# xXCoffeeColaXc/WeatherConverter

Hardware: NVIDIA B200
Metric: guided translation images/sec (256x512, T steps) at 1/2/4/8 B200 vs host CPU (higher is better)
Workload: dtype bf16

## Files before the change

### include/wc_b200.h

```cpp
#ifndef WC_B200_H_
#define WC_B200_H_

#include <stddef.h>
#include <stdint.h>

#ifdef __cplusplus
extern "C" {
#endif

typedef uint16_t wc_bf16;

const char* wc_last_error(void);
int wc_abi_version(void);
long long wc_launch_count(void);

void wc_profile_begin(void);
int wc_profile_end(double* ms_by_class, long long* count_by_class, double* work_by_class);
int wc_profile_detail(int cap, int* cls, double* ms, double* work, int* info);

int wc_ddpm_step(const float* xt, const float* eps, const float* z, float* out, float* mean_out, float* sigz_out,
                 size_t n_per_sample, int batch, float beta, float sqrt_one_minus_acp, float sqrt_alpha, float sigma,
                 void* stream);
int wc_ddpm_step_batched(const float* xt, const float* eps, const float* z, float* out, float* mean_out,
                         float* sigz_out, size_t n_per_sample, int batch, const float* betas, const float* alphas,
                         const float* sqrt_one_minus_acp, const int64_t* t, int num_timesteps, void* stream);
int wc_ddpm_step_indexed(const float* xt, const float* eps, const float* z, float* out, float* mean_out, float* sigz_out,
                         size_t n_per_sample, int batch, const float* coef_tables, const int64_t* t_dev, int num_timesteps,
                         void* stream);
int wc_ddim_step(const float* xt, const float* eps, const float* z, float* out, float* mean_out, float* sigz_out,
                 size_t n_per_sample, int batch, float a_t, float s_t, float a_prev, float d, float sigma, void* stream);
int wc_ddim_step_indexed(const float* xt, const float* eps, const float* z, float* out, float* mean_out, float* sigz_out,
                         size_t n_per_sample, int batch, const float* coef_tables, const int64_t* t_dev, int num_timesteps,
                         void* stream);
int wc_add_noise(const float* x0, const float* noise, float* out, size_t n_per_sample, int batch,
                 const float* sqrt_acp, const float* sqrt_one_minus_acp, const int64_t* t, int num_timesteps, void* stream);

int wc_set_time_factor_table(const float* factor_host, int half);
int wc_time_embedding(const int64_t* t, int n, int dim, float* out, void* stream);

int wc_sgg_update(const float* grad, const float* mu, const float* sigz, float* out, float* mag_out, int batch, int h,
                  int w, int pool, float lambda, void* stream);

int wc_lcg_prepare(const float* sr_xt, const int64_t* gt, float* x_masked, int64_t* gt_masked, int batch, int num_classes,
                   int H, int W, void* stream);
int wc_lcg_combine(const float* pooled_grads, const int64_t* gt, const float* mu, const float* sigz, float* out, int batch,
                   int num_classes, int h, int w, int pool, float lambda, void* stream);

size_t wc_groupnorm_workspace_bytes(int batch);
int wc_groupnorm_silu(const wc_bf16* x, wc_bf16* y, int batch, int hw, int channels, int ldx, int ldy,
                      const float* gamma, const float* beta, float eps, int silu, void* workspace, void* stream);
int wc_conv2d(const wc_bf16* x, int batch, int H, int W, int Cin, int ldx, const float* weight, const float* bias,
              int Cout, int K, int stride, int pad, int dil, int transposed, const float* rowbias,
              const wc_bf16* residual, int ldr, const wc_bf16* x2, int Cin2, int ldx2, const float* weight2, int relu,
              wc_bf16* y, int ldy, void* stream);
int wc_conv_in(const float* x, const float* weight, const float* bias, const float* scale, const float* shift,
               wc_bf16* y, int batch, int H, int W, int Cout, int K, int stride, int pad, int ldy, int relu,
               void* stream);
int wc_conv_out(const wc_bf16* x, const float* weight, const float* bias, float* y, int batch, int H, int W, int Cin,
                int K, int ldx, int tanh_out, void* stream);
int wc_conv2d_dgrad(const wc_bf16* dz, int batch, int Ho, int Wo, int Cout, const float* weight, int Cin, int K, int stride,
                    int dil, const wc_bf16* residual, const wc_bf16* mask, wc_bf16* dx, void* stream);
int wc_maxpool3x3s2(const wc_bf16* x, wc_bf16* y, uint8_t* idx, int batch, int H, int W, int C, void* stream);
int wc_maxpool3x3s2_bwd(const wc_bf16* dy, const uint8_t* idx, const wc_bf16* x, wc_bf16* dx, int batch, int H, int W, int C,
                        void* stream);
int wc_bilinear(const wc_bf16* x, wc_bf16* y, int batch, int Hi, int Wi, int Ho, int Wo, int C, void* stream);
int wc_bilinear_bwd(const wc_bf16* dy, const wc_bf16* mask, wc_bf16* dx, int batch, int Hi, int Wi, int Ho, int Wo, int C,
                    void* stream);
int wc_seg_loss_head(const float* logits_lo, const int64_t* labels, int* n_valid_ws, int64_t* pred, float* dlogit_hi,
                     float* loss, float* logits_hi, wc_bf16* dlogit_lo, int batch, int h, int w, int H, int W, void* stream);
int wc_conv1_dgrad(const wc_bf16* dz, const float* weight, const float* scale, float* dx, int batch, int H, int W, void* stream);
int wc_nchw_f32_to_nhwc_bf16(const float* x, wc_bf16* y, int batch, int C, int hw, int ldy, void* stream);
int wc_nhwc_bf16_to_nchw_f32(const wc_bf16* x, float* y, int batch, int C, int hw, int ldx, void* stream);
int wc_attention(const wc_bf16* q, const wc_bf16* k, const wc_bf16* vt, wc_bf16* out, int batch, int heads, int ntok,
                 int hd, int ldo, void* stream);
int wc_attention_scaled(const wc_bf16* q, const wc_bf16* k, const wc_bf16* vt, wc_bf16* out, int batch, int heads, int ntok,
                        int hd, int ldo, float scale, void* stream);

int wc_ddpm_grid_u8(const float* x, uint8_t* out, int batch, int H, int W, int nrow, int padding, void* stream);
int wc_postprocess_u8(const float* x, uint8_t* out, int batch, int H, int W, const float* mean3_host, const float* std3_host, void* stream);
int wc_label_encode(const uint8_t* label_ids, int Ws, const int* ytab, const int* xtab, int top, int left, int Hc, int Wc,
                    const int64_t* lut, int nlut, int64_t* out, void* stream);
int wc_resample_u8(const uint8_t* in, uint8_t* tmp, uint8_t* out, int Hin, int Win, int Hout, int Wout, int channels, const int* bounds_h,
                   const int* kk_h, int ksize_h, const int* bounds_v, const int* kk_v, int ksize_v, void* stream);
int wc_u8_to_tensor(const uint8_t* in, int Win, int top, int left, int Hc, int Wc, int mode, const float* mean3_host, const float* std3_host,
                    float* out, void* stream);

int wc_attention_lse(const wc_bf16* q, const wc_bf16* k, const wc_bf16* vt, wc_bf16* out, float* lse, int batch, int heads,
                     int ntok, int hd, int ldo, void* stream);
int wc_attention_bwd(const wc_bf16* q, const wc_bf16* k, const wc_bf16* v, const wc_bf16* o, const wc_bf16* d_o, const float* lse,
                     float* d_scratch, wc_bf16* dqkv, int batch, int heads, int ntok, int hd, void* stream);
int wc_conv2d_wgrad(const wc_bf16* x, const wc_bf16* dy, int batch, int H, int W, int Cin, int Cout, int K, int stride, int pad,
                    int dil, int transposed, const wc_bf16* x2, int Cin2, float* dw, float* dw2, void* stream);
size_t wc_groupnorm_bwd_workspace_bytes(int batch, int channels);
int wc_groupnorm_silu_bwd(const wc_bf16* x, const wc_bf16* dy, wc_bf16* dx, int batch, int hw, int channels, const float* gamma,
                          const float* beta, float eps, int silu, const void* fwd_workspace, const wc_bf16* add1,
                          const wc_bf16* add2, float* dgamma, float* dbeta, void* workspace, void* stream);
int wc_colsum(const wc_bf16* x, int batch, int hw, int channels, float* out_rows, float* out_total, void* workspace, void* stream);
int wc_mse_loss_grad(const float* pred, const float* target, float* dpred, size_t n, float grad_scale, float* loss, void* scratch,
                     void* stream);
size_t wc_boundary_wgrad_scratch_bytes(void);
int wc_boundary_wgrad(const wc_bf16* wide, const float* narrow, int batch, int H, int W, int sign, float* dw, float* dbias,
                      void* scratch, void* stream);
int wc_adam_step(float* p, const float* g, float* m, float* v, size_t n, float lr, float beta1, float beta2, float eps, int step,
                 float grad_scale, void* stream);

typedef struct wc_unet wc_unet;
typedef struct {
  int im_channels, im_size, time_emb_dim, num_down_layers, num_mid_layers, num_up_layers, num_heads;
  int n_down_channels;
  int down_channels[8];
  int n_mid_channels;
  int mid_channels[8];
  int down_sample[8];
  int n_attn_resolutions;
  int attn_resolutions[8];
} wc_unet_config;
int wc_unet_create(wc_unet** out, const wc_unet_config* cfg, int n_params, const char* const* names,
                   const float* const* ptrs, const int64_t* numels, void* stream);
void wc_unet_destroy(wc_unet* net);
size_t wc_unet_workspace_bytes(const wc_unet* net, int batch, int H, int W);
int wc_unet_forward(wc_unet* net, const float* x, const int64_t* t, int n_t, float* out, int batch, int H, int W,
                    void* workspace, size_t workspace_bytes, void* stream);
double wc_unet_flops(const wc_unet* net);
int wc_unet_launches(const wc_unet* net);

typedef struct wc_unet_train wc_unet_train;
int wc_unet_train_create(wc_unet_train** out, const wc_unet_config* cfg, int n_params, const char* const* names,
                         float* const* params, float* const* grads);
void wc_unet_train_destroy(wc_unet_train* net);
size_t wc_unet_train_workspace_bytes(wc_unet_train* net, int batch, int H, int W);
int wc_unet_train_bind(wc_unet_train* net, int batch, int H, int W, void* workspace, size_t workspace_bytes, void* stream);
int wc_unet_train_forward(wc_unet_train* net, const float* x, const int64_t* t, const float* target, float* pred_out,
                          float* loss_out, float grad_scale, int repack, void* stream);
int wc_unet_train_num_backward_ops(const wc_unet_train* net);
int wc_unet_train_backward(wc_unet_train* net, int op_begin, int op_end, void* stream);
int wc_unet_train_backward_seeded(wc_unet_train* net, const float* dpred, float* dx, int param_grads, void* stream);
int wc_unet_train_grad_ready_op(const wc_unet_train* net, const char* name);
double wc_unet_train_flops(const wc_unet_train* net, int backward);

typedef struct wc_legacy_unet wc_legacy_unet;
int wc_legacy_unet_create(wc_legacy_unet** out, int n_params, const char* const* names, const float* const* ptrs,
                          const int64_t* numels);
void wc_legacy_unet_destroy(wc_legacy_unet* net);
size_t wc_legacy_unet_workspace_bytes(wc_legacy_unet* net, int batch, int size);
int wc_legacy_unet_forward(wc_legacy_unet* net, const float* x, const float* t, float* out, int batch, int size, void* workspace,
                           size_t workspace_bytes, void* stream);
double wc_legacy_unet_flops(const wc_legacy_unet* net);
int wc_legacy_unet_launches(const wc_legacy_unet* net);

typedef struct wc_seg wc_seg;
int wc_seg_create(wc_seg** out, const int* blocks_per_layer, int num_classes, int n_params, const char* const* names,
                  const float* const* ptrs, void* stream);
int wc_seg_set_output_stride(wc_seg* net, int output_stride);
void wc_seg_destroy(wc_seg* net);
size_t wc_seg_workspace_bytes(const wc_seg* net, int batch, int H, int W, int with_grad);
int wc_seg_infer(wc_seg* net, const float* x, const int64_t* labels, int64_t* pred, float* input_grad, float* loss,
                 float* logits, int batch, int H, int W, void* workspace, size_t workspace_bytes, void* stream);
int wc_seg_infer_pooled(wc_seg* net, const float* x, const int64_t* labels, int64_t* pred, float* input_grad, float* loss,
                        float* logits, int batch, int H, int W, int grad_pool, void* workspace, size_t workspace_bytes,
                        void* stream);
int wc_seg_forward(wc_seg* net, const float* x, float* logits, int batch, int H, int W, int save_for_backward, void* workspace,
                   size_t workspace_bytes, void* stream);
int wc_seg_backward_seeded(wc_seg* net, const float* dlogits, float* input_grad, void* stream);
double wc_seg_flops(const wc_seg* net, int backward);
int wc_seg_launches(const wc_seg* net);

typedef struct wc_srgan wc_srgan;
int wc_srgan_create(wc_srgan** out, int num_blocks, int upscale, int n_params, const char* const* names,
                    const float* const* ptrs, void* stream);
void wc_srgan_destroy(wc_srgan* net);
size_t wc_srgan_workspace_bytes(const wc_srgan* net, int batch, int h, int w);
int wc_srgan_forward(wc_srgan* net, const float* x, float* y, int batch, int h, int w, void* workspace,
                     size_t workspace_bytes, void* stream);
size_t wc_srgan_grad_workspace_bytes(const wc_srgan* net, int batch, int h, int w);
int wc_srgan_forward_saved(wc_srgan* net, const float* x, float* y, int batch, int h, int w, void* workspace,
                           size_t workspace_bytes, void* stream);
int wc_srgan_backward_seeded(wc_srgan* net, const float* dy, float* dx, void* stream);
double wc_srgan_flops(const wc_srgan* net);
int wc_srgan_launches(const wc_srgan* net);

#ifdef __cplusplus
}
#endif
#endif
```

### weatherconverter_b200/_lib.py

```python
import ctypes as C
import os

import torch

_HERE = os.path.dirname(os.path.abspath(__file__))
LIB_PATH = os.path.join(_HERE, "libwc_b200.so")

_lib = None

c_f32p = C.c_void_p
c_ptr = C.c_void_p


class UnetConfigStruct(C.Structure):
    _fields_ = [
        ("im_channels", C.c_int), ("im_size", C.c_int), ("time_emb_dim", C.c_int),
        ("num_down_layers", C.c_int), ("num_mid_layers", C.c_int), ("num_up_layers", C.c_int),
        ("num_heads", C.c_int),
        ("n_down_channels", C.c_int), ("down_channels", C.c_int * 8),
        ("n_mid_channels", C.c_int), ("mid_channels", C.c_int * 8),
        ("down_sample", C.c_int * 8),
        ("n_attn_resolutions", C.c_int), ("attn_resolutions", C.c_int * 8),
    ]


_SIGS = {
    "wc_last_error": (C.c_char_p, []),
    "wc_abi_version": (C.c_int, []),
    "wc_launch_count": (C.c_longlong, []),
    "wc_profile_begin": (None, []),
    "wc_profile_detail": (C.c_int, [C.c_int, C.POINTER(C.c_int), C.POINTER(C.c_double), C.POINTER(C.c_double), C.POINTER(C.c_int)]),
    "wc_profile_end": (C.c_int, [C.POINTER(C.c_double), C.POINTER(C.c_longlong), C.POINTER(C.c_double)]),
    "wc_ddpm_step": (C.c_int, [c_ptr] * 6 + [C.c_size_t, C.c_int] + [C.c_float] * 4 + [c_ptr]),
    "wc_ddpm_step_batched": (C.c_int, [c_ptr] * 6 + [C.c_size_t, C.c_int] + [c_ptr] * 4 + [C.c_int, c_ptr]),
    "wc_ddpm_step_indexed": (C.c_int, [c_ptr] * 6 + [C.c_size_t, C.c_int, c_ptr, c_ptr, C.c_int, c_ptr]),
    "wc_ddim_step": (C.c_int, [c_ptr] * 6 + [C.c_size_t, C.c_int] + [C.c_float] * 5 + [c_ptr]),
    "wc_ddim_step_indexed": (C.c_int, [c_ptr] * 6 + [C.c_size_t, C.c_int, c_ptr, c_ptr, C.c_int, c_ptr]),
    "wc_add_noise": (C.c_int, [c_ptr] * 3 + [C.c_size_t, C.c_int] + [c_ptr] * 3 + [C.c_int, c_ptr]),
    "wc_set_time_factor_table": (C.c_int, [C.POINTER(C.c_float), C.c_int]),
    "wc_time_embedding": (C.c_int, [c_ptr, C.c_int, C.c_int, c_ptr, c_ptr]),
    "wc_sgg_update": (C.c_int, [c_ptr] * 5 + [C.c_int] * 4 + [C.c_float, c_ptr]),
    "wc_lcg_prepare": (C.c_int, [c_ptr] * 4 + [C.c_int] * 4 + [c_ptr]),
    "wc_lcg_combine": (C.c_int, [c_ptr] * 5 + [C.c_int] * 5 + [C.c_float, c_ptr]),
    "wc_groupnorm_workspace_bytes": (C.c_size_t, [C.c_int]),
    "wc_groupnorm_silu": (C.c_int, [c_ptr, c_ptr] + [C.c_int] * 5 + [c_ptr, c_ptr, C.c_float, C.c_int, c_ptr, c_ptr]),
    "wc_conv2d": (C.c_int, [c_ptr] + [C.c_int] * 5 + [c_ptr, c_ptr] + [C.c_int] * 6 + [c_ptr, c_ptr, C.c_int, c_ptr,
                            C.c_int, C.c_int, c_ptr, C.c_int, c_ptr, C.c_int, c_ptr]),
    "wc_conv2d_dgrad": (C.c_int, [c_ptr] + [C.c_int] * 4 + [c_ptr] + [C.c_int] * 4 + [c_ptr] * 4),
    "wc_maxpool3x3s2": (C.c_int, [c_ptr] * 3 + [C.c_int] * 4 + [c_ptr]),
    "wc_maxpool3x3s2_bwd": (C.c_int, [c_ptr] * 4 + [C.c_int] * 4 + [c_ptr]),
    "wc_bilinear": (C.c_int, [c_ptr] * 2 + [C.c_int] * 6 + [c_ptr]),
    "wc_bilinear_bwd": (C.c_int, [c_ptr] * 3 + [C.c_int] * 6 + [c_ptr]),
    "wc_seg_loss_head": (C.c_int, [c_ptr] * 8 + [C.c_int] * 5 + [c_ptr]),
    "wc_conv1_dgrad": (C.c_int, [c_ptr] * 4 + [C.c_int] * 3 + [c_ptr]),
    "wc_conv_in": (C.c_int, [c_ptr] * 6 + [C.c_int] * 9 + [c_ptr]),
    "wc_conv_out": (C.c_int, [c_ptr] * 4 + [C.c_int] * 7 + [c_ptr]),
    "wc_nchw_f32_to_nhwc_bf16": (C.c_int, [c_ptr, c_ptr] + [C.c_int] * 4 + [c_ptr]),
    "wc_nhwc_bf16_to_nchw_f32": (C.c_int, [c_ptr, c_ptr] + [C.c_int] * 4 + [c_ptr]),
    "wc_attention": (C.c_int, [c_ptr] * 4 + [C.c_int] * 5 + [c_ptr]),
    "wc_ddpm_grid_u8": (C.c_int, [c_ptr, c_ptr] + [C.c_int] * 5 + [c_ptr]),
    "wc_postprocess_u8": (C.c_int, [c_ptr, c_ptr] + [C.c_int] * 3 + [C.POINTER(C.c_float), C.POINTER(C.c_float), c_ptr]),
    "wc_label_encode": (C.c_int, [c_ptr, C.c_int, c_ptr, c_ptr] + [C.c_int] * 4 + [c_ptr, C.c_int, c_ptr, c_ptr]),
    "wc_resample_u8": (C.c_int, [c_ptr] * 3 + [C.c_int] * 5 + [c_ptr, c_ptr, C.c_int, c_ptr, c_ptr, C.c_int, c_ptr]),
    "wc_u8_to_tensor": (C.c_int, [c_ptr] + [C.c_int] * 6 + [C.POINTER(C.c_float), C.POINTER(C.c_float), c_ptr, c_ptr]),
    "wc_attention_lse": (C.c_int, [c_ptr] * 5 + [C.c_int] * 5 + [c_ptr]),
    "wc_attention_scaled": (C.c_int, [c_ptr] * 4 + [C.c_int] * 5 + [C.c_float, c_ptr]),
    "wc_attention_bwd": (C.c_int, [c_ptr] * 8 + [C.c_int] * 4 + [c_ptr]),
    "wc_conv2d_wgrad": (C.c_int, [c_ptr, c_ptr] + [C.c_int] * 10 + [c_ptr, C.c_int, c_ptr, c_ptr, c_ptr]),
    "wc_groupnorm_bwd_workspace_bytes": (C.c_size_t, [C.c_int, C.c_int]),
    "wc_groupnorm_silu_bwd": (C.c_int, [c_ptr] * 3 + [C.c_int] * 3 + [c_ptr, c_ptr, C.c_float, C.c_int] + [c_ptr] * 7),
    "wc_colsum": (C.c_int, [c_ptr] + [C.c_int] * 3 + [c_ptr] * 4),
    "wc_mse_loss_grad": (C.c_int, [c_ptr] * 3 + [C.c_size_t, C.c_float, c_ptr, c_ptr, c_ptr]),
    "wc_boundary_wgrad_scratch_bytes": (C.c_size_t, []),
    "wc_boundary_wgrad": (C.c_int, [c_ptr, c_ptr] + [C.c_int] * 4 + [c_ptr] * 4),
    "wc_adam_step": (C.c_int, [c_ptr] * 4 + [C.c_size_t] + [C.c_float] * 4 + [C.c_int, C.c_float, c_ptr]),
    "wc_unet_create": (C.c_int, [C.POINTER(c_ptr), C.POINTER(UnetConfigStruct), C.c_int, C.POINTER(C.c_char_p),
                                 C.POINTER(c_ptr), C.POINTER(C.c_int64), c_ptr]),
    "wc_unet_destroy": (None, [c_ptr]),
    "wc_unet_workspace_bytes": (C.c_size_t, [c_ptr, C.c_int, C.c_int, C.c_int]),
    "wc_unet_forward": (C.c_int, [c_ptr, c_ptr, c_ptr, C.c_int, c_ptr, C.c_int, C.c_int, C.c_int, c_ptr, C.c_size_t,
                                  c_ptr]),
    "wc_unet_flops": (C.c_double, [c_ptr]),
    "wc_unet_launches": (C.c_int, [c_ptr]),
    "wc_unet_train_create": (C.c_int, [C.POINTER(c_ptr), C.POINTER(UnetConfigStruct), C.c_int, C.POINTER(C.c_char_p),
                                       C.POINTER(c_ptr), C.POINTER(c_ptr)]),
    "wc_unet_train_destroy": (None, [c_ptr]),
    "wc_unet_train_workspace_bytes": (C.c_size_t, [c_ptr, C.c_int, C.c_int, C.c_int]),
    "wc_unet_train_bind": (C.c_int, [c_ptr, C.c_int, C.c_int, C.c_int, c_ptr, C.c_size_t, c_ptr]),
    "wc_unet_train_forward": (C.c_int, [c_ptr] * 6 + [C.c_float, C.c_int, c_ptr]),
    "wc_unet_train_num_backward_ops": (C.c_int, [c_ptr]),
    "wc_unet_train_backward": (C.c_int, [c_ptr, C.c_int, C.c_int, c_ptr]),
    "wc_unet_train_backward_seeded": (C.c_int, [c_ptr, c_ptr, c_ptr, C.c_int, c_ptr]),
    "wc_unet_train_grad_ready_op": (C.c_int, [c_ptr, C.c_char_p]),
    "wc_unet_train_flops": (C.c_double, [c_ptr, C.c_int]),
    "wc_legacy_unet_create": (C.c_int, [C.POINTER(c_ptr), C.c_int, C.POINTER(C.c_char_p), C.POINTER(c_ptr), C.POINTER(C.c_int64)]),
    "wc_legacy_unet_destroy": (None, [c_ptr]),
    "wc_legacy_unet_workspace_bytes": (C.c_size_t, [c_ptr, C.c_int, C.c_int]),
    "wc_legacy_unet_forward": (C.c_int, [c_ptr, c_ptr, c_ptr, c_ptr, C.c_int, C.c_int, c_ptr, C.c_size_t, c_ptr]),
    "wc_legacy_unet_flops": (C.c_double, [c_ptr]),
    "wc_legacy_unet_launches": (C.c_int, [c_ptr]),
    "wc_seg_create": (C.c_int, [C.POINTER(c_ptr), C.POINTER(C.c_int), C.c_int, C.c_int, C.POINTER(C.c_char_p),
                                C.POINTER(c_ptr), c_ptr]),
    "wc_seg_set_output_stride": (C.c_int, [c_ptr, C.c_int]),
    "wc_seg_destroy": (None, [c_ptr]),
    "wc_seg_workspace_bytes": (C.c_size_t, [c_ptr, C.c_int, C.c_int, C.c_int, C.c_int]),
    "wc_seg_infer": (C.c_int, [c_ptr] * 7 + [C.c_int] * 3 + [c_ptr, C.c_size_t, c_ptr]),
    "wc_seg_infer_pooled": (C.c_int, [c_ptr] * 7 + [C.c_int] * 4 + [c_ptr, C.c_size_t, c_ptr]),
    "wc_seg_forward": (C.c_int, [c_ptr] * 3 + [C.c_int] * 4 + [c_ptr, C.c_size_t, c_ptr]),
    "wc_seg_backward_seeded": (C.c_int, [c_ptr] * 4),
    "wc_seg_flops": (C.c_double, [c_ptr, C.c_int]),
    "wc_seg_launches": (C.c_int, [c_ptr]),
    "wc_srgan_create": (C.c_int, [C.POINTER(c_ptr), C.c_int, C.c_int, C.c_int, C.POINTER(C.c_char_p), C.POINTER(c_ptr), c_ptr]),
    "wc_srgan_destroy": (None, [c_ptr]),
    "wc_srgan_workspace_bytes": (C.c_size_t, [c_ptr, C.c_int, C.c_int, C.c_int]),
    "wc_srgan_forward": (C.c_int, [c_ptr, c_ptr, c_ptr, C.c_int, C.c_int, C.c_int, c_ptr, C.c_size_t, c_ptr]),
    "wc_srgan_grad_workspace_bytes": (C.c_size_t, [c_ptr, C.c_int, C.c_int, C.c_int]),
    "wc_srgan_forward_saved": (C.c_int, [c_ptr, c_ptr, c_ptr, C.c_int, C.c_int, C.c_int, c_ptr, C.c_size_t, c_ptr]),
    "wc_srgan_backward_seeded": (C.c_int, [c_ptr] * 4),
    "wc_srgan_flops": (C.c_double, [c_ptr]),
    "wc_srgan_launches": (C.c_int, [c_ptr]),
}

EXPORTS = tuple(_SIGS.keys())


def lib():
    global _lib
    if _lib is None:
        if not os.path.exists(LIB_PATH):
            raise RuntimeError(
                f"{LIB_PATH} not found: the CUDA extension has not been built "
                "(run __graft_entry__.build()); this package has no CPU fallback")
        handle = C.CDLL(LIB_PATH)
        for name, (res, args) in _SIGS.items():
            fn = getattr(handle, name)
            fn.restype = res
            fn.argtypes = args
        _lib = handle
    return _lib


def check(rc):
    if rc != 0:
        msg = lib().wc_last_error()
        raise RuntimeError("wc_b200: " + (msg.decode() if msg else f"error {rc}"))


def require_cuda(*tensors):
    if not torch.cuda.is_available():
        raise RuntimeError("wc_b200 needs a CUDA device (sm_100a); there is no CPU fallback")
    for t in tensors:
        if t is not None and not t.is_cuda:
            raise RuntimeError("wc_b200 kernels take CUDA tensors; got a tensor on " + str(t.device))


def ptr(t):
    return None if t is None else C.c_void_p(t.data_ptr())


def stream_ptr():
    return C.c_void_p(torch.cuda.current_stream().cuda_stream)
```

### weatherconverter_b200/csrc/seg.cu

```cuda
#include "plan.cuh"
#include "../../include/wc_b200.h"

namespace wc {
int conv_small_cin(const float* x, const float* w, const float* bias, const float* scale, const float* shift,
                   __nv_bfloat16* y, int B, int Cin, int H, int W, int Cout, int K, int stride, int pad, int ldy,
                   int relu, cudaStream_t st, const float* prelu = nullptr);
int bn_fold(const float* g, const float* b, const float* mean, const float* var, float eps, float* scale, float* shift,
            int n, int n_pad, cudaStream_t st);
int maxpool_fwd(const __nv_bfloat16* x, __nv_bfloat16* y, uint8_t* idx, int B, int H, int W, int C, cudaStream_t st);
int maxpool_bwd(const __nv_bfloat16* dy, const uint8_t* idx, const __nv_bfloat16* x, __nv_bfloat16* dx, int B, int H,
                int W, int C, cudaStream_t st);
int gap_fwd(const __nv_bfloat16* x, __nv_bfloat16* y, int B, int HW, int C, int ld, cudaStream_t st);
int broadcast_hw(const __nv_bfloat16* v, __nv_bfloat16* y, int B, int HW, int C, int ldy, cudaStream_t st);
int sum_hw(const __nv_bfloat16* y, const __nv_bfloat16* mask, __nv_bfloat16* v, int B, int HW, int C, int ldy, cudaStream_t st);
int gap_bwd_add(const __nv_bfloat16* g, __nv_bfloat16* dx, int B, int HW, int C, int ld, cudaStream_t st);
int bilinear_fwd(const __nv_bfloat16* x, __nv_bfloat16* y, int B, int Hi, int Wi, int Ho, int Wo, int C, int ldx, int ldy,
                 cudaStream_t st);
int bilinear_bwd(const __nv_bfloat16* dy, const __nv_bfloat16* mask, __nv_bfloat16* dx, int B, int Hi, int Wi, int Ho,
                 int Wo, int C, int ldy, int ldm, int ldx, cudaStream_t st);
int seg_loss_grad(const float* logits_lo, const long long* labels, int* n_valid, long long* pred, float* dlogit_hi,
                  float* loss, float* logits_hi, int B, int h, int w, int H, int W, int nc, int ignore, cudaStream_t st);
int seg_loss_head_fused(const float* logits_lo, const long long* labels, int* n_valid, long long* pred, float* loss,
                        __nv_bfloat16* dlo, int B, int h, int w, int H, int W, int nc, int cp, int ldo, int ignore, cudaStream_t st);
int logits_bilinear_bwd(const float* dhi, __nv_bfloat16* dlo, int B, int h, int w, int H, int W, int nc, int cp, int ldo,
                        cudaStream_t st);
int conv1_dgrad(const __nv_bfloat16* dz, const float* w, const float* scale, float* dx, int B, int H, int W, int Cout,
                cudaStream_t st);
int relu_mask_inplace(__nv_bfloat16* d, const __nv_bfloat16* m, size_t npix, int C, int ldd, int ldm, cudaStream_t st);
int conv1_dgrad_weff(const float* w, const float* scale, float* weff, int P, cudaStream_t st);
int conv1_dgrad_pooled(const __nv_bfloat16* dz, const float* weff, float* out, int B, int H, int W, int P, cudaStream_t st);
}

struct wc_seg {
  int layers[4];
  int num_classes;
  int output_stride = 16;
  wc::ParamTable params;
  std::unique_ptr<wc::DeviceArena> arena;
  int B = 0, H = 0, W = 0, with_grad = 0, grad_pool = 1;
  void* ws = nullptr;
  size_t ws_bytes = 0;
  wc::OpList fwd_ops, bwd_ops;
  double flops_fwd = 0, flops_bwd = 0;
  size_t ws_needed = 0;
  size_t n_body_ops = 0;
  float* logits_lo = nullptr;
  __nv_bfloat16* dlo = nullptr;
  int saved_fwd = 0;
  const float* x_in = nullptr;
  const long long* labels = nullptr;
  long long* pred = nullptr;
  float* grad_out = nullptr;
  float* loss = nullptr;
  float* logits_hi = nullptr;
};

namespace wc {
namespace {

struct BlockRec {
  std::string p;
  int inplanes, planes, stride, dil;
  bool has_down;
  Act x_in, y1, y2, out;
};

struct SegBuilder {
  wc_seg* net;
  Bump bump;
  DeviceArena* arena;
  cudaStream_t st;
  bool dry;
  int B;
  int err = 0;
  bool in_bwd = false;
  std::unordered_map<std::string, std::pair<float*, float*>> bn;

  const float* P(const std::string& n) { return net->params.get(n, &err); }
  void push(std::function<int(cudaStream_t)> f) {
    if (dry) return;
    (in_bwd ? net->bwd_ops : net->fwd_ops).push_back(std::move(f));
  }
  Act act(int H, int W, int C) { return make_act(bump, B, H, W, C); }

  std::pair<float*, float*> bnfold(const std::string& prefix, int C) {
    auto it = bn.find(prefix);
    if (it != bn.end()) return it->second;
    const int cp = (C + 15) / 16 * 16;
    float* sc = static_cast<float*>(arena->alloc(cp * sizeof(float)));
    float* sh = static_cast<float*>(arena->alloc(cp * sizeof(float)));
    const float *g = P(prefix + ".weight"), *b = P(prefix + ".bias"), *m = P(prefix + ".running_mean"), *v = P(prefix + ".running_var");
    if (!sc || !sh || err) { if (!err) err = 1; return {nullptr, nullptr}; }
    if (int e = bn_fold(g, b, m, v, 1e-5f, sc, sh, C, cp, st)) err = e;
    bn[prefix] = {sc, sh};
    return {sc, sh};
  }

  void conv_bn(const Act& x, const std::string& wname, const std::string& bnname, int cin, int cout, int K, int stride,
               int dil, const Act* res, int relu, const Act& out) {
    if (dry) return;
    auto sb = bnfold(bnname, cout);
    WeightSrc w; w.w = P(wname + ".weight"); w.d0 = cout; w.d1 = cin; w.KH = w.KW = K; w.scale = sb.first;
    if (err) return;
    ConvGeom g; g.K = K; g.stride = stride; g.dil = dil;
    g.pad = (stride == 1) ? dil * (K - 1) / 2 : (K == 3 ? 1 : 0);
    Epilogue ep; ep.bias = sb.second; ep.res = res; ep.relu = relu;
    OutSpec os; os.mode = kOutNHWC; os.out = out;
    auto op = std::make_shared<ConvOp>();
    if (int e = build_conv(op.get(), arena, x, w, g, cout, nullptr, nullptr, ep, os, st)) { err = e; return; }
    net->flops_fwd += op->flops;
    push([op](cudaStream_t s) { return op->run(s); });
  }

  void dgrad(const Act& dz, const std::string& wname, const std::string& bnname, int cin, int cout, int K, int stride,
             int dil, const Act* res, const Act* mask, const Act& dx, const float* scale_override = nullptr, bool no_bn = false) {
    if (dry) return;
    const float* sc = no_bn ? scale_override : bnfold(bnname, cout).first;
    WeightSrc w; w.w = P(wname + ".weight"); w.d0 = cout; w.d1 = cin; w.KH = w.KW = K; w.transpose = 1; w.scale = sc;
    if (err) return;
    Epilogue ep; ep.res = res; ep.mask = mask;
    OutSpec os; os.mode = kOutNHWC; os.out = dx;
    auto op = std::make_shared<ConvOp>();
    int e;
    if (stride == 1) {
      w.flip = 1;
      ConvGeom g; g.K = K; g.stride = 1; g.dil = dil; g.pad = dil * (K - 1) / 2;
      e = build_conv(op.get(), arena, dz, w, g, cin, nullptr, nullptr, ep, os, st);
    } else {
      e = build_conv_transposed_s2(op.get(), arena, dz, w, K, K == 3 ? 1 : 0, cin, ep, os, st);
    }
    if (e) { err = e; return; }
    net->flops_bwd += op->flops;
    push([op](cudaStream_t s) { return op->run(s); });
  }
};

int build(wc_seg* net, bool dry, void* ws, size_t ws_bytes, cudaStream_t st) {
  const int B = net->B, H = net->H, W = net->W, NC = net->num_classes;
  SegBuilder b{net, dry ? Bump::dry() : Bump(ws, ws_bytes), net->arena.get(), st, dry, B};
  const int H2 = H / 2, W2 = W / 2, H4 = H / 4, W4 = W / 4;
  Act c1 = b.act(H2, W2, 64);
  Act p1 = b.act(H4, W4, 64);
  uint8_t* pool_idx = static_cast<uint8_t*>(b.bump.take(p1.pixels() * 64));
  static int stem_tc = -1;
  if (stem_tc < 0) {
    const char* e = getenv("WC_SEG_STEM_TC");
    stem_tc = e ? atoi(e) : 1;
  }
  const bool tc_stem = stem_tc && H % 2 == 0 && W % 2 == 0;
  __nv_bfloat16* xpad = tc_stem ? static_cast<__nv_bfloat16*>(b.bump.take(static_cast<size_t>(B) * H * (W + 8) * 8 * sizeof(__nv_bfloat16))) : nullptr;
  std::pair<float*, float*> bn1{nullptr, nullptr};
  const float* w_conv1 = nullptr;
  if (!dry) {
    bn1 = b.bnfold("backbone.bn1", 64);
    w_conv1 = b.P("backbone.conv1.weight");
    if (b.err) return b.err;
    wc_seg* n = net;
    const float *sc = bn1.first, *sh = bn1.second;
    if (tc_stem) {
      float* wprime = static_cast<float*>(b.arena->alloc(64 * 64 * 7 * sizeof(float)));
      if (!wprime) return 1;
      if (int e = stem_weights(w_conv1, wprime, 64, st)) return e;
      Epilogue ep; ep.bias = sh; ep.relu = 1;
      OutSpec os; os.mode = kOutNHWC; os.out = c1;
      auto op = std::make_shared<ConvOp>();
      if (int e = build_conv_stem7s2(op.get(), b.arena, xpad, B, H, W, wprime, sc, 64, ep, os, st)) return e;
      b.push([=](cudaStream_t s) {
        if (int e = stem_prepare(n->x_in, xpad, B, H, W, s)) return e;
        if (int e = op->run(s)) return e;
        return maxpool_fwd(c1.ptr, p1.ptr, pool_idx, B, H2, W2, 64, s);
      });
    } else {
      b.push([=](cudaStream_t s) {
        if (int e = conv_small_cin(n->x_in, w_conv1, nullptr, sc, sh, c1.ptr, B, 3, H, W, 64, 7, 2, 3, 64, 1, s)) return e;
        return maxpool_fwd(c1.ptr, p1.ptr, pool_idx, B, H2, W2, 64, s);
      });
    }
    net->flops_fwd += 2.0 * B * H2 * W2 * 147.0 * 64;
  }
  std::vector<BlockRec> blocks;
  {
    int inplanes = 64, dilation = 1;
    const int planes_l[4] = {64, 128, 256, 512}, stride_l[4] = {1, 2, 2, 2};
    const bool os8 = net->output_stride == 8;
    const bool dilate_l[4] = {false, false, os8, true};
    for (int li = 0; li < 4; ++li) {
      const int prev = dilation;
      int stride = stride_l[li];
      if (dilate_l[li]) { dilation *= stride; stride = 1; }
      for (int bi = 0; bi < net->layers[li]; ++bi) {
        BlockRec r;
        r.p = "backbone.layer" + std::to_string(li + 1) + "." + std::to_string(bi);
        r.inplanes = inplanes; r.planes = planes_l[li];
        r.stride = bi == 0 ? stride : 1;
        r.dil = bi == 0 ? prev : dilation;
        r.has_down = bi == 0 && (stride != 1 || inplanes != planes_l[li] * 4);
        blocks.push_back(r);
        inplanes = planes_l[li] * 4;
      }
    }
  }
  Act cur = p1;
  Act low;
  for (size_t i = 0; i < blocks.size(); ++i) {
    BlockRec& r = blocks[i];
    r.x_in = cur;
    const int Ho = cur.H / r.stride, Wo = cur.W / r.stride;
    r.y1 = b.act(cur.H, cur.W, r.planes);
    b.conv_bn(cur, r.p + ".conv1", r.p + ".bn1", r.inplanes, r.planes, 1, 1, 1, nullptr, 1, r.y1);
    r.y2 = b.act(Ho, Wo, r.planes);
    b.conv_bn(r.y1, r.p + ".conv2", r.p + ".bn2", r.planes, r.planes, 3, r.stride, r.dil, nullptr, 1, r.y2);
    Act idt = cur;
    if (r.has_down) {
      idt = b.act(Ho, Wo, r.planes * 4);
      b.conv_bn(cur, r.p + ".downsample.0", r.p + ".downsample.1", r.inplanes, r.planes * 4, 1, r.stride, 1, nullptr, 0, idt);
    }
    r.out = b.act(Ho, Wo, r.planes * 4);
    b.conv_bn(r.y2, r.p + ".conv3", r.p + ".bn3", r.planes, r.planes * 4, 1, 1, 1, &idt, 1, r.out);
    cur = r.out;
    if (static_cast<int>(i) + 1 == net->layers[0]) low = cur;
    if (b.err) return b.err;
  }
  const Act feat = cur;
  const int h = feat.H, w = feat.W;
  const std::string c = "classifier";
  Act cat5 = b.act(h, w, 1280);
  b.conv_bn(feat, c + ".aspp.convs.0.0", c + ".aspp.convs.0.1", 2048, 256, 1, 1, 1, nullptr, 1, slice_act(cat5, 0, 256));
  const int rmul = net->output_stride == 8 ? 2 : 1;
  const int rates[3] = {6 * rmul, 12 * rmul, 18 * rmul};
  for (int k = 0; k < 3; ++k)
    b.conv_bn(feat, c + ".aspp.convs." + std::to_string(k + 1) + ".0", c + ".aspp.convs." + std::to_string(k + 1) + ".1", 2048,
              256, 3, 1, rates[k], nullptr, 1, slice_act(cat5, 256 * (k + 1), 256));
  Act pooled = b.act(1, 1, 2048), g2 = b.act(1, 1, 256);
  b.push([=](cudaStream_t s) { return gap_fwd(feat.ptr, pooled.ptr, B, h * w, 2048, feat.ld, s); });
  b.conv_bn(pooled, c + ".aspp.convs.4.1", c + ".aspp.convs.4.2", 2048, 256, 1, 1, 1, nullptr, 1, g2);
  {
    Act dst = slice_act(cat5, 1024, 256);
    b.push([=](cudaStream_t s) { return broadcast_hw(g2.ptr, dst.ptr, B, h * w, 256, dst.ld, s); });
  }
  Act aspp = b.act(h, w, 256);
  b.conv_bn(cat5, c + ".aspp.project.0", c + ".aspp.project.1", 1280, 256, 1, 1, 1, nullptr, 1, aspp);
  Act cat2 = b.act(H4, W4, 304);
  Act ll = slice_act(cat2, 0, 48), up = slice_act(cat2, 48, 256);
  b.conv_bn(low, c + ".project.0", c + ".project.1", 256, 48, 1, 1, 1, nullptr, 1, ll);
  b.push([=](cudaStream_t s) { return bilinear_fwd(aspp.ptr, up.ptr, B, h, w, H4, W4, 256, aspp.ld, up.ld, s); });
  Act y = b.act(H4, W4, 256);
  b.conv_bn(cat2, c + ".classifier.0", c + ".classifier.1", 304, 256, 3, 1, 1, nullptr, 1, y);
  const int NCP = 32;
  float* logits_lo = static_cast<float*>(b.bump.take(static_cast<size_t>(B) * NC * H4 * W4 * sizeof(float)));
  if (!dry) {
    float* bias_pad = static_cast<float*>(b.arena->alloc(NCP * sizeof(float)));
    const float* bias = b.P(c + ".classifier.3.bias");
    WeightSrc wsrc; wsrc.w = b.P(c + ".classifier.3.weight"); wsrc.d0 = NC; wsrc.d1 = 256;
    if (!bias_pad || b.err) return b.err ? b.err : 1;
    WC_CHECK_CUDA(cudaMemsetAsync(bias_pad, 0, NCP * sizeof(float), st));
    WC_CHECK_CUDA(cudaMemcpyAsync(bias_pad, bias, NC * sizeof(float), cudaMemcpyDeviceToDevice, st));
    ConvGeom g; g.K = 1; g.pad = 0;
    Epilogue ep; ep.bias = bias_pad;
    OutSpec os; os.mode = kOutNCHWf32; os.out_f32 = logits_lo; os.n_store = NC;
    auto op = std::make_shared<ConvOp>();
    if (int e = build_conv(op.get(), b.arena, y, wsrc, g, NCP, nullptr, nullptr, ep, os, st)) return e;
    net->flops_fwd += op->flops;
    b.push([op](cudaStream_t s) { return op->run(s); });
  }
  float* dlogit_hi = static_cast<float*>(b.bump.take(static_cast<size_t>(B) * H * W * NC * sizeof(float)));
  int* n_valid = static_cast<int*>(b.bump.take(B * sizeof(int)));
  static int loss_fused = -1;
  if (loss_fused < 0) {
    const char* e = getenv("WC_SEG_LOSS_FUSED");
    loss_fused = e ? atoi(e) : 1;
  }
  Act dlo{};
  if (net->with_grad) dlo = b.act(H4, W4, NCP);
  if (!dry) {
    net->n_body_ops = net->fwd_ops.size();
    net->logits_lo = logits_lo;
    net->dlo = net->with_grad ? dlo.ptr : nullptr;
  }
  {
    wc_seg* n = net;
    const bool with_grad = net->with_grad;
    const int fused = loss_fused;
    b.push([=](cudaStream_t s) {
      if (with_grad && fused && !n->logits_hi) {
        const int e = seg_loss_head_fused(logits_lo, n->labels, n_valid, n->pred, n->loss, dlo.ptr, B, H4, W4, H, W, NC, NCP, NCP, 255, s);
        if (e != -1) return e;
      }
      if (int e = seg_loss_grad(logits_lo, n->labels, n_valid, n->pred, dlogit_hi, n->loss, n->logits_hi, B, H4, W4, H, W, NC, 255, s)) return e;
      return with_grad ? logits_bilinear_bwd(dlogit_hi, dlo.ptr, B, H4, W4, H, W, NC, NCP, NCP, s) : 0;
    });
  }
  if (!net->with_grad) {
    if (dry) net->ws_needed = b.bump.used() + 4096;
    else if (b.bump.overflow()) return fail("seg workspace too small");
    return b.err;
  }
  b.in_bwd = true;
  Act dlo19 = dlo; dlo19.C = NC;
  Act dy = b.act(H4, W4, 256);
  b.dgrad(dlo19, c + ".classifier.3", "", 256, NC, 1, 1, 1, nullptr, &y, dy, nullptr, true);
  Act dcat2 = b.act(H4, W4, 304);
  b.dgrad(dy, c + ".classifier.0", c + ".classifier.1", 304, 256, 3, 1, 1, nullptr, nullptr, dcat2);
  Act d_ll = slice_act(dcat2, 0, 48), d_up = slice_act(dcat2, 48, 256);
  b.push([=](cudaStream_t s) { return relu_mask_inplace(d_ll.ptr, ll.ptr, d_ll.pixels(), 48, d_ll.ld, ll.ld, s); });
  Act dlow_extra = b.act(H4, W4, 256);
  b.dgrad(d_ll, c + ".project.0", c + ".project.1", 256, 48, 1, 1, 1, nullptr, nullptr, dlow_extra);
  Act daspp = b.act(h, w, 256);
  b.push([=](cudaStream_t s) {
    return bilinear_bwd(d_up.ptr, aspp.ptr, daspp.ptr, B, h, w, H4, W4, 256, d_up.ld, aspp.ld, daspp.ld, s);
  });
  Act dcat5 = b.act(h, w, 1280);
  b.dgrad(daspp, c + ".aspp.project.0", c + ".aspp.project.1", 1280, 256, 1, 1, 1, nullptr, &cat5, dcat5);
  Act dfeat = b.act(h, w, 2048);
  {
    Act d0 = slice_act(dcat5, 0, 256);
    b.dgrad(d0, c + ".aspp.convs.0.0", c + ".aspp.convs.0.1", 2048, 256, 1, 1, 1, nullptr, nullptr, dfeat);
    for (int k = 0; k < 3; ++k) {
      Act dk = slice_act(dcat5, 256 * (k + 1), 256);
      b.dgrad(dk, c + ".aspp.convs." + std::to_string(k + 1) + ".0", c + ".aspp.convs." + std::to_string(k + 1) + ".1", 2048, 256,
              3, 1, rates[k], &dfeat, nullptr, dfeat);
    }
    Act d4 = slice_act(dcat5, 1024, 256);
    Act dg2 = b.act(1, 1, 256), dpooled = b.act(1, 1, 2048);
    b.push([=](cudaStream_t s) { return sum_hw(d4.ptr, nullptr, dg2.ptr, B, h * w, 256, d4.ld, s); });
    b.dgrad(dg2, c + ".aspp.convs.4.1", c + ".aspp.convs.4.2", 2048, 256, 1, 1, 1, nullptr, nullptr, dpooled);
    b.push([=](cudaStream_t s) {
      if (int e = gap_bwd_add(dpooled.ptr, dfeat.ptr, B, h * w, 2048, dfeat.ld, s)) return e;
      return relu_mask_inplace(dfeat.ptr, feat.ptr, dfeat.pixels(), 2048, dfeat.ld, feat.ld, s);
    });
  }
  Act g = dfeat;
  for (int i = static_cast<int>(blocks.size()) - 1; i >= 0; --i) {
    const BlockRec& r = blocks[i];
    const bool first_block = (i == 0);
    const bool feeds_low = (i == net->layers[0]);
    Act d2 = b.act(g.H, g.W, r.planes);
    b.dgrad(g, r.p + ".conv3", r.p + ".bn3", r.planes, r.planes * 4, 1, 1, 1, nullptr, &r.y2, d2);
    Act d1 = b.act(r.x_in.H, r.x_in.W, r.planes);
    b.dgrad(d2, r.p + ".conv2", r.p + ".bn2", r.planes, r.planes, 3, r.stride, r.dil, nullptr, &r.y1, d1);
    Act didt = g;
    if (r.has_down) {
      didt = b.act(r.x_in.H, r.x_in.W, r.inplanes);
      const size_t bytes = didt.pixels() * didt.C * sizeof(__nv_bfloat16);
      const bool need_init = (r.stride == 2) || feeds_low;
      if (need_init) {
        if (feeds_low) {
          b.push([=](cudaStream_t s) {
            return cudaMemcpyAsync(didt.ptr, dlow_extra.ptr, bytes, cudaMemcpyDeviceToDevice, s) == cudaSuccess ? 0 : fail("memcpy failed");
          });
        } else {
          b.push([=](cudaStream_t s) { return cudaMemsetAsync(didt.ptr, 0, bytes, s) == cudaSuccess ? 0 : fail("memset failed"); });
        }
      }
      b.dgrad(g, r.p + ".downsample.0", r.p + ".downsample.1", r.inplanes, r.planes * 4, 1, r.stride, 1, need_init ? &didt : nullptr,
              nullptr, didt);
    } else if (feeds_low) {
      return fail("internal: the block after layer1 is expected to have a downsample branch");
    }
    Act dx = b.act(r.x_in.H, r.x_in.W, r.inplanes);
    b.dgrad(d1, r.p + ".conv1", r.p + ".bn1", r.inplanes, r.planes, 1, 1, 1, &didt, first_block ? nullptr : &r.x_in, dx);
    g = dx;
    if (b.err) return b.err;
  }
  Act dc1 = b.act(H2, W2, 64);
  {
    wc_seg* n = net;
    const Act gp = g;
    const float* sc = bn1.first;
    const int P = net->grad_pool;
    float* weff = nullptr;
    if (!dry && P > 1) {
      const int R = P / 2 + 3;
      weff = static_cast<float*>(b.arena->alloc(static_cast<size_t>(R) * R * 192 * sizeof(float)));
      if (!weff) return 1;
      if (int e = conv1_dgrad_weff(w_conv1, sc, weff, P, st)) return e;
    }
    b.push([=](cudaStream_t s) {
      if (int e = maxpool_bwd(gp.ptr, pool_idx, c1.ptr, dc1.ptr, B, H2, W2, 64, s)) return e;
      if (P > 1) return conv1_dgrad_pooled(dc1.ptr, weff, n->grad_out, B, H, W, P, s);
      return conv1_dgrad(dc1.ptr, w_conv1, sc, n->grad_out, B, H, W, 64, s);
    });
    net->flops_bwd += 2.0 * B * H2 * W2 * 147.0 * 64;
  }
  if (dry) net->ws_needed = b.bump.used() + 4096;
  else if (b.bump.overflow()) return fail("seg workspace too small: need " + std::to_string(b.bump.used()) + " bytes");
  return b.err;
}

int bind_plan(wc_seg* net, int batch, int H, int W, int with_grad, int grad_pool, void* workspace, size_t workspace_bytes,
              cudaStream_t st) {
  if (net->B == batch && net->H == H && net->W == W && net->with_grad == with_grad && net->grad_pool == grad_pool && net->ws == workspace &&
      net->ws_bytes == workspace_bytes)
    return 0;
  net->fwd_ops.clear(); net->bwd_ops.clear();
  net->arena = std::make_unique<DeviceArena>();
  net->B = batch; net->H = H; net->W = W; net->with_grad = with_grad; net->grad_pool = grad_pool; net->ws = workspace; net->ws_bytes = workspace_bytes;
  net->flops_fwd = net->flops_bwd = 0;
  if (int e = build(net, false, workspace, workspace_bytes, st)) {
    net->B = 0;
    net->fwd_ops.clear(); net->bwd_ops.clear();
    return e;
  }
  return 0;
}

}
}

using namespace wc;

extern "C" {

int wc_seg_create(wc_seg** out, const int* blocks_per_layer, int num_classes, int n_params, const char* const* names,
                  const float* const* ptrs, void* stream) {
  (void)stream;
  WC_REQUIRE(out && blocks_per_layer && names && ptrs, "null argument");
  WC_REQUIRE(num_classes == 19, "the loss head is built for 19 classes");
  auto net = std::make_unique<wc_seg>();
  for (int i = 0; i < 4; ++i) net->layers[i] = blocks_per_layer[i];
  net->num_classes = num_classes;
  for (int i = 0; i < n_params; ++i) net->params.ptr[names[i]] = ptrs[i];
  *out = net.release();
  return 0;
}

int wc_seg_set_output_stride(wc_seg* net, int output_stride) {
  WC_REQUIRE(net, "null handle");
  WC_REQUIRE(output_stride == 8 || output_stride == 16, "output_stride must be 8 or 16 (modeling.py:34-39)");
  if (net->output_stride != output_stride) {
    net->output_stride = output_stride;
    net->B = net->H = net->W = 0;
    net->saved_fwd = 0;
  }
  return 0;
}

void wc_seg_destroy(wc_seg* net) { delete net; }

size_t wc_seg_workspace_bytes(const wc_seg* net_c, int batch, int H, int W, int with_grad) {
  wc_seg* net = const_cast<wc_seg*>(net_c);
  const int sB = net->B, sH = net->H, sW = net->W, sg = net->with_grad;
  net->B = batch; net->H = H; net->W = W; net->with_grad = with_grad;
  size_t need = 0;
  if (build(net, true, nullptr, 0, nullptr) == 0) need = net->ws_needed;
  net->B = sB; net->H = sH; net->W = sW; net->with_grad = sg;
  return need;
}

int wc_seg_infer_pooled(wc_seg* net, const float* x, const int64_t* labels, int64_t* pred, float* input_grad, float* loss,
                        float* logits, int batch, int H, int W, int grad_pool, void* workspace, size_t workspace_bytes,
                        void* stream);

int wc_seg_infer(wc_seg* net, const float* x, const int64_t* labels, int64_t* pred, float* input_grad, float* loss,
                 float* logits, int batch, int H, int W, void* workspace, size_t workspace_bytes, void* stream) {
  return wc_seg_infer_pooled(net, x, labels, pred, input_grad, loss, logits, batch, H, W, 1, workspace, workspace_bytes, stream);
}

int wc_seg_infer_pooled(wc_seg* net, const float* x, const int64_t* labels, int64_t* pred, float* input_grad, float* loss,
                        float* logits, int batch, int H, int W, int grad_pool, void* workspace, size_t workspace_bytes,
                        void* stream) {
  if (net) net->saved_fwd = 0;
  WC_REQUIRE(grad_pool >= 1, "grad_pool must be >= 1");
  WC_REQUIRE(net && x && labels && workspace, "null argument");
  WC_REQUIRE(H % 32 == 0 && W % 32 == 0, "H and W must be multiples of 32 (output stride 16, stride-2 phase views)");
  cudaStream_t st = static_cast<cudaStream_t>(stream);
  const int with_grad = input_grad != nullptr;
  if (int e = bind_plan(net, batch, H, W, with_grad, grad_pool, workspace, workspace_bytes, st)) return e;
  net->x_in = x; net->labels = reinterpret_cast<const long long*>(labels);
  net->pred = reinterpret_cast<long long*>(pred); net->grad_out = input_grad; net->loss = loss; net->logits_hi = logits;
  for (auto& op : net->fwd_ops)
    if (int e = op(st)) return e;
  for (auto& op : net->bwd_ops)
    if (int e = op(st)) return e;
  return 0;
}

int wc_seg_forward(wc_seg* net, const float* x, float* logits, int batch, int H, int W, int save_for_backward, void* workspace,
                   size_t workspace_bytes, void* stream) {
  if (net) net->saved_fwd = 0;
  WC_REQUIRE(net && x && logits && workspace, "null argument");
  WC_REQUIRE(H % 32 == 0 && W % 32 == 0, "H and W must be multiples of 32 (output stride 16, stride-2 phase views)");
  cudaStream_t st = static_cast<cudaStream_t>(stream);
  if (int e = bind_plan(net, batch, H, W, save_for_backward ? 1 : 0, 1, workspace, workspace_bytes, st)) return e;
  net->x_in = x; net->labels = nullptr; net->pred = nullptr; net->grad_out = nullptr; net->loss = nullptr; net->logits_hi = logits;
  for (size_t i = 0; i < net->n_body_ops; ++i)
    if (int e = net->fwd_ops[i](st)) return e;
  if (int e = seg_loss_grad(net->logits_lo, nullptr, nullptr, nullptr, nullptr, nullptr, logits, batch, H / 4, W / 4, H, W,
                            net->num_classes, 255, st))
    return e;
  net->saved_fwd = save_for_backward ? 1 : 0;
  return 0;
}

int wc_seg_backward_seeded(wc_seg* net, const float* dlogits, float* input_grad, void* stream) {
  WC_REQUIRE(net && dlogits && input_grad, "null argument");
  WC_REQUIRE(net->saved_fwd && net->dlo,
             "wc_seg_backward_seeded: this handle holds no saved forward; the last call on it must be "
             "wc_seg_forward(save_for_backward = 1) (an infer or another forward in between discards the saved activations)");
  net->saved_fwd = 0;
  cudaStream_t st = static_cast<cudaStream_t>(stream);
  const int B = net->B, H = net->H, W = net->W;
  net->grad_out = input_grad;
  if (int e = logits_bilinear_bwd(dlogits, net->dlo, B, H / 4, W / 4, H, W, net->num_classes, 32, 32, st)) return e;
  for (auto& op : net->bwd_ops)
    if (int e = op(st)) return e;
  return 0;
}

double wc_seg_flops(const wc_seg* net, int backward) { return net ? (backward ? net->flops_bwd : net->flops_fwd) : 0.0; }
int wc_seg_launches(const wc_seg* net) { return net ? static_cast<int>(net->fwd_ops.size() + net->bwd_ops.size()) : 0; }

}
```

### weatherconverter_b200/csrc/seg_kernels.cu

```cuda
#include <cuda_fp16.h>
#include <cstdlib>
#include "wc_host.h"
#include "wc_ptx.cuh"

namespace wc {

namespace {

inline int grid_for(size_t n_items, int per_block = 256) {
  const size_t blocks = (n_items + per_block - 1) / per_block;
  const size_t cap = static_cast<size_t>(num_sms()) * 16;
  return static_cast<int>(blocks < cap ? (blocks ? blocks : 1) : cap);
}

__global__ void bn_fold_kernel(const float* g, const float* b, const float* mean, const float* var, float eps,
                               float* scale, float* shift, int n, int n_pad) {
  pdl_prologue();
  const int i = blockIdx.x * blockDim.x + threadIdx.x;
  if (i >= n_pad) return;
  if (i < n) {
    const float s = g[i] / sqrtf(var[i] + eps);
    scale[i] = s;
    shift[i] = b[i] - mean[i] * s;
  } else {
    scale[i] = 0.f;
    shift[i] = 0.f;
  }
}

__global__ void maxpool_fwd_kernel(const __nv_bfloat16* __restrict__ x, __nv_bfloat16* __restrict__ y,
                                   uint8_t* __restrict__ idx, int B, int H, int W, int C, int Ho, int Wo) {
  pdl_prologue();
  const int c8n = C / 8;
  const size_t total = static_cast<size_t>(B) * Ho * Wo * c8n;
  for (size_t i = blockIdx.x * static_cast<size_t>(blockDim.x) + threadIdx.x; i < total;
       i += static_cast<size_t>(gridDim.x) * blockDim.x) {
    const int c8 = static_cast<int>(i % c8n);
    size_t p = i / c8n;
    const int ox = static_cast<int>(p % Wo), oy = static_cast<int>((p / Wo) % Ho), b = static_cast<int>(p / (static_cast<size_t>(Wo) * Ho));
    float best[8];
    int bi[8];
#pragma unroll
    for (int j = 0; j < 8; ++j) { best[j] = -INFINITY; bi[j] = 0; }
    for (int ky = 0; ky < 3; ++ky) {
      const int iy = oy * 2 - 1 + ky;
      if (iy < 0 || iy >= H) continue;
      for (int kx = 0; kx < 3; ++kx) {
        const int ix = ox * 2 - 1 + kx;
        if (ix < 0 || ix >= W) continue;
        const uint4 u = __ldg(reinterpret_cast<const uint4*>(x + ((static_cast<size_t>(b) * H + iy) * W + ix) * C + c8 * 8));
        float f[8];
        float2 t;
        t = unpack_bf16(u.x); f[0] = t.x; f[1] = t.y;
        t = unpack_bf16(u.y); f[2] = t.x; f[3] = t.y;
        t = unpack_bf16(u.z); f[4] = t.x; f[5] = t.y;
        t = unpack_bf16(u.w); f[6] = t.x; f[7] = t.y;
#pragma unroll
        for (int j = 0; j < 8; ++j)
          if (f[j] > best[j]) { best[j] = f[j]; bi[j] = ky * 3 + kx; }
      }
    }
    uint4 o;
    o.x = pack_bf16(best[0], best[1]); o.y = pack_bf16(best[2], best[3]);
    o.z = pack_bf16(best[4], best[5]); o.w = pack_bf16(best[6], best[7]);
    *reinterpret_cast<uint4*>(y + p * C + c8 * 8) = o;
    uint2 ii;
    ii.x = bi[0] | (bi[1] << 8) | (bi[2] << 16) | (bi[3] << 24);
    ii.y = bi[4] | (bi[5] << 8) | (bi[6] << 16) | (bi[7] << 24);
    *reinterpret_cast<uint2*>(idx + p * C + c8 * 8) = ii;
  }
}

__global__ void maxpool_bwd_kernel(const __nv_bfloat16* __restrict__ dy, const uint8_t* __restrict__ idx,
                                   const __nv_bfloat16* __restrict__ x, __nv_bfloat16* __restrict__ dx, int B, int H,
                                   int W, int C, int Ho, int Wo) {
  pdl_prologue();
  const int c8n = C / 8;
  const size_t total = static_cast<size_t>(B) * H * W * c8n;
  for (size_t i = blockIdx.x * static_cast<size_t>(blockDim.x) + threadIdx.x; i < total;
       i += static_cast<size_t>(gridDim.x) * blockDim.x) {
    const int c8 = static_cast<int>(i % c8n);
    size_t p = i / c8n;
    const int ix = static_cast<int>(p % W), iy = static_cast<int>((p / W) % H), b = static_cast<int>(p / (static_cast<size_t>(W) * H));
    float acc[8];
#pragma unroll
    for (int j = 0; j < 8; ++j) acc[j] = 0.f;
    for (int oy = iy / 2; oy <= (iy + 1) / 2; ++oy) {
      if (oy >= Ho) continue;
      const int ky = iy - (2 * oy - 1);
      for (int ox = ix / 2; ox <= (ix + 1) / 2; ++ox) {
        if (ox >= Wo) continue;
        const int kx = ix - (2 * ox - 1);
        const uint32_t tap = static_cast<uint32_t>(ky * 3 + kx);
        const size_t q = ((static_cast<size_t>(b) * Ho + oy) * Wo + ox) * C + c8 * 8;
        const uint2 ii = __ldg(reinterpret_cast<const uint2*>(idx + q));
        const uint4 g = __ldg(reinterpret_cast<const uint4*>(dy + q));
        const uint32_t* gp = &g.x;
#pragma unroll
        for (int j = 0; j < 8; ++j) {
          const uint32_t t = ((j < 4 ? ii.x : ii.y) >> (8 * (j & 3))) & 0xffu;
          const float2 f = unpack_bf16(gp[j >> 1]);
          if (t == tap) acc[j] += (j & 1) ? f.y : f.x;
        }
      }
    }
    const uint4 xv = __ldg(reinterpret_cast<const uint4*>(x + p * C + c8 * 8));
    const uint32_t* xp = &xv.x;
    uint32_t o[4];
#pragma unroll
    for (int j = 0; j < 4; ++j) {
      const float2 f = unpack_bf16(xp[j]);
      o[j] = pack_bf16(f.x > 0.f ? acc[2 * j] : 0.f, f.y > 0.f ? acc[2 * j + 1] : 0.f);
    }
    *reinterpret_cast<uint4*>(dx + p * C + c8 * 8) = make_uint4(o[0], o[1], o[2], o[3]);
  }
}

__global__ void gap_fwd_kernel(const __nv_bfloat16* __restrict__ x, __nv_bfloat16* __restrict__ y, int HW, int C, int ld) {
  pdl_prologue();
  __shared__ float red[4][64];
  const int b = blockIdx.y, c = blockIdx.x * 64 + (threadIdx.x & 63), part = threadIdx.x >> 6;
  float acc = 0.f;
  if (c < C)
    for (int p = part; p < HW; p += 4) acc += __bfloat162float(x[(static_cast<size_t>(b) * HW + p) * ld + c]);
  red[part][threadIdx.x & 63] = acc;
  __syncthreads();
  if (part == 0 && c < C)
    y[static_cast<size_t>(b) * C + c] = __float2bfloat16_rn((red[0][threadIdx.x] + red[1][threadIdx.x] + red[2][threadIdx.x] + red[3][threadIdx.x]) / HW);
}
__global__ void broadcast_kernel(const __nv_bfloat16* __restrict__ v, __nv_bfloat16* __restrict__ y, int B, int HW, int C, int ldy) {
  pdl_prologue();
  const int c8n = C / 8;
  const size_t total = static_cast<size_t>(B) * HW * c8n;
  for (size_t i = blockIdx.x * static_cast<size_t>(blockDim.x) + threadIdx.x; i < total;
       i += static_cast<size_t>(gridDim.x) * blockDim.x) {
    const int c8 = static_cast<int>(i % c8n);
    const size_t p = i / c8n, b = p / HW;
    *reinterpret_cast<uint4*>(y + p * ldy + c8 * 8) = __ldg(reinterpret_cast<const uint4*>(v + b * C + c8 * 8));
  }
}
__global__ void sum_hw_kernel(const __nv_bfloat16* __restrict__ y, const __nv_bfloat16* __restrict__ m,
                              __nv_bfloat16* __restrict__ v, int HW, int C, int ldy) {
  pdl_prologue();
  __shared__ float red[4][64];
  const int b = blockIdx.y, c = blockIdx.x * 64 + (threadIdx.x & 63), part = threadIdx.x >> 6;
  float acc = 0.f;
  if (c < C)
    for (int p = part; p < HW; p += 4) acc += __bfloat162float(y[(static_cast<size_t>(b) * HW + p) * ldy + c]);
  red[part][threadIdx.x & 63] = acc;
  __syncthreads();
  if (part == 0 && c < C) {
    float s = red[0][threadIdx.x] + red[1][threadIdx.x] + red[2][threadIdx.x] + red[3][threadIdx.x];
    if (m && !(__bfloat162float(m[static_cast<size_t>(b) * C + c]) > 0.f)) s = 0.f;
    v[static_cast<size_t>(b) * C + c] = __float2bfloat16_rn(s);
  }
}
__global__ void gap_bwd_add_kernel(const __nv_bfloat16* __restrict__ g, __nv_bfloat16* __restrict__ dx, int B, int HW, int C, int ld) {
  pdl_prologue();
  const size_t total = static_cast<size_t>(B) * HW * C;
  const float inv = 1.f / HW;
  for (size_t i = blockIdx.x * static_cast<size_t>(blockDim.x) + threadIdx.x; i < total;
       i += static_cast<size_t>(gridDim.x) * blockDim.x) {
    const int c = static_cast<int>(i % C);
    const size_t p = i / C, b = p / HW;
    __nv_bfloat16* d = dx + p * ld + c;
    *d = __float2bfloat16_rn(__bfloat162float(*d) + __bfloat162float(g[b * C + c]) * inv);
  }
}

__device__ __forceinline__ void bilinear_src(int dst, float scale, int in_size, int& i0, int& i1, float& l1) {
  float src = (dst + 0.5f) * scale - 0.5f;
  if (src < 0.f) src = 0.f;
  i0 = static_cast<int>(src);
  if (i0 > in_size - 1) i0 = in_size - 1;
  i1 = i0 + (i0 < in_size - 1 ? 1 : 0);
  l1 = src - i0;
}

__global__ void bilinear_fwd_kernel(const __nv_bfloat16* __restrict__ x, __nv_bfloat16* __restrict__ y, int B, int Hi,
                                    int Wi, int Ho, int Wo, int C, int ldx, int ldy) {
  pdl_prologue();
  const int c8n = C / 8;
  const size_t total = static_cast<size_t>(B) * Ho * Wo * c8n;
  const float sy = static_cast<float>(Hi) / Ho, sx = static_cast<float>(Wi) / Wo;
  for (size_t i = blockIdx.x * static_cast<size_t>(blockDim.x) + threadIdx.x; i < total;
       i += static_cast<size_t>(gridDim.x) * blockDim.x) {
    const int c8 = static_cast<int>(i % c8n);
    size_t p = i / c8n;
    const int ox = static_cast<int>(p % Wo), oy = static_cast<int>((p / Wo) % Ho), b = static_cast<int>(p / (static_cast<size_t>(Wo) * Ho));
    int y0, y1, x0, x1;
    float ly, lx;
    bilinear_src(oy, sy, Hi, y0, y1, ly);
    bilinear_src(ox, sx, Wi, x0, x1, lx);
    const float w00 = (1.f - ly) * (1.f - lx), w01 = (1.f - ly) * lx, w10 = ly * (1.f - lx), w11 = ly * lx;
    const __nv_bfloat16* xb = x + static_cast<size_t>(b) * Hi * Wi * ldx + c8 * 8;
    const uint4 a = __ldg(reinterpret_cast<const uint4*>(xb + (static_cast<size_t>(y0) * Wi + x0) * ldx));
    const uint4 bq = __ldg(reinterpret_cast<const uint4*>(xb + (static_cast<size_t>(y0) * Wi + x1) * ldx));
    const uint4 c = __ldg(reinterpret_cast<const uint4*>(xb + (static_cast<size_t>(y1) * Wi + x0) * ldx));
    const uint4 d = __ldg(reinterpret_cast<const uint4*>(xb + (static_cast<size_t>(y1) * Wi + x1) * ldx));
    const uint32_t* pa = &a.x; const uint32_t* pb = &bq.x; const uint32_t* pc = &c.x; const uint32_t* pd = &d.x;
    uint32_t o[4];
#pragma unroll
    for (int j = 0; j < 4; ++j) {
      const float2 fa = unpack_bf16(pa[j]), fb = unpack_bf16(pb[j]), fc = unpack_bf16(pc[j]), fd = unpack_bf16(pd[j]);
      o[j] = pack_bf16(w00 * fa.x + w01 * fb.x + w10 * fc.x + w11 * fd.x, w00 * fa.y + w01 * fb.y + w10 * fc.y + w11 * fd.y);
    }
    *reinterpret_cast<uint4*>(y + p * ldy + c8 * 8) = make_uint4(o[0], o[1], o[2], o[3]);
  }
}

__global__ void bilinear_bwd_kernel(const __nv_bfloat16* __restrict__ dy, const __nv_bfloat16* __restrict__ m,
                                    __nv_bfloat16* __restrict__ dx, int B, int Hi, int Wi, int Ho, int Wo, int C,
                                    int ldy, int ldm, int ldx) {
  pdl_prologue();
  const int c8n = C / 8;
  const size_t total = static_cast<size_t>(B) * Hi * Wi * c8n;
  const float sy = static_cast<float>(Hi) / Ho, sx = static_cast<float>(Wi) / Wo;
  const int fy = (Ho + Hi - 1) / Hi, fx = (Wo + Wi - 1) / Wi;
  for (size_t i = blockIdx.x * static_cast<size_t>(blockDim.x) + threadIdx.x; i < total;
       i += static_cast<size_t>(gridDim.x) * blockDim.x) {
    const int c8 = static_cast<int>(i % c8n);
    size_t p = i / c8n;
    const int ix = static_cast<int>(p % Wi), iy = static_cast<int>((p / Wi) % Hi), b = static_cast<int>(p / (static_cast<size_t>(Wi) * Hi));
    float acc[8];
#pragma unroll
    for (int j = 0; j < 8; ++j) acc[j] = 0.f;
    const int oy_lo = max(0, fy * iy - fy - 1), oy_hi = min(Ho - 1, fy * iy + 2 * fy);
    const int ox_lo = max(0, fx * ix - fx - 1), ox_hi = min(Wo - 1, fx * ix + 2 * fx);
    for (int oy = oy_lo; oy <= oy_hi; ++oy) {
      int y0, y1; float ly;
      bilinear_src(oy, sy, Hi, y0, y1, ly);
      float wy = 0.f;
      if (y0 == iy) wy += 1.f - ly;
      if (y1 == iy) wy += ly;
      if (wy == 0.f) continue;
      for (int ox = ox_lo; ox <= ox_hi; ++ox) {
        int x0, x1; float lx;
        bilinear_src(ox, sx, Wi, x0, x1, lx);
        float wx = 0.f;
        if (x0 == ix) wx += 1.f - lx;
        if (x1 == ix) wx += lx;
        if (wx == 0.f) continue;
        const float ww = wy * wx;
        const uint4 u = __ldg(reinterpret_cast<const uint4*>(dy + ((static_cast<size_t>(b) * Ho + oy) * Wo + ox) * ldy + c8 * 8));
        const uint32_t* up = &u.x;
#pragma unroll
        for (int j = 0; j < 4; ++j) {
          const float2 f = unpack_bf16(up[j]);
          acc[2 * j] = fmaf(ww, f.x, acc[2 * j]);
          acc[2 * j + 1] = fmaf(ww, f.y, acc[2 * j + 1]);
        }
      }
    }
    if (m) {
      const uint4 mv = __ldg(reinterpret_cast<const uint4*>(m + p * ldm + c8 * 8));
      const uint32_t* mp = &mv.x;
#pragma unroll
      for (int j = 0; j < 4; ++j) {
        const float2 f = unpack_bf16(mp[j]);
        if (!(f.x > 0.f)) acc[2 * j] = 0.f;
        if (!(f.y > 0.f)) acc[2 * j + 1] = 0.f;
      }
    }
    uint4 o;
    o.x = pack_bf16(acc[0], acc[1]); o.y = pack_bf16(acc[2], acc[3]); o.z = pack_bf16(acc[4], acc[5]); o.w = pack_bf16(acc[6], acc[7]);
    *reinterpret_cast<uint4*>(dx + p * ldx + c8 * 8) = o;
  }
}

__global__ void count_valid_kernel(const long long* __restrict__ labels, int HW, int ignore, int* __restrict__ n_valid) {
  pdl_prologue();
  const int b = blockIdx.y;
  int cnt = 0;
  for (int p = blockIdx.x * blockDim.x + threadIdx.x; p < HW; p += gridDim.x * blockDim.x)
    cnt += labels[static_cast<size_t>(b) * HW + p] != ignore;
  cnt = __reduce_add_sync(0xffffffffu, cnt);
  if ((threadIdx.x & 31) == 0 && cnt) atomicAdd(n_valid + b, cnt);
}

template <int NC>
__global__ void seg_loss_grad_kernel(const float* __restrict__ logits_lo, const long long* __restrict__ labels,
                                     const int* __restrict__ n_valid, long long* __restrict__ pred,
                                     float* __restrict__ dlogit_hi, float* __restrict__ loss, float* __restrict__ logits_hi,
                                     int B, int h, int w, int H, int W, int ignore) {
  pdl_prologue();
  const size_t total = static_cast<size_t>(B) * H * W;
  const float sy = static_cast<float>(h) / H, sx = static_cast<float>(w) / W;
  const size_t lane = threadIdx.x & 31;
  for (size_t wb = (blockIdx.x * static_cast<size_t>(blockDim.x) + threadIdx.x) - lane; wb < total;
       wb += static_cast<size_t>(gridDim.x) * blockDim.x) {
    const size_t i = wb + lane;
    float lsum = 0.f;
    int b = 0;
    if (i < total) {
      const int ox = static_cast<int>(i % W), oy = static_cast<int>((i / W) % H);
      b = static_cast<int>(i / (static_cast<size_t>(W) * H));
      int y0, y1, x0, x1;
      float ly, lx;
      bilinear_src(oy, sy, h, y0, y1, ly);
      bilinear_src(ox, sx, w, x0, x1, lx);
      const float w00 = (1.f - ly) * (1.f - lx), w01 = (1.f - ly) * lx, w10 = ly * (1.f - lx), w11 = ly * lx;
      const size_t plane = static_cast<size_t>(h) * w;
      const float* lb = logits_lo + static_cast<size_t>(b) * NC * plane;
      float v[NC];
      float mx = -INFINITY;
      int am = 0;
#pragma unroll
      for (int c = 0; c < NC; ++c) {
        const float* pl = lb + c * plane;
        v[c] = w00 * pl[y0 * w + x0] + w01 * pl[y0 * w + x1] + w10 * pl[y1 * w + x0] + w11 * pl[y1 * w + x1];
        if (v[c] > mx) { mx = v[c]; am = c; }
      }
      if (pred) pred[i] = am;
      if (logits_hi) {
        const size_t pl_hi = static_cast<size_t>(H) * W;
#pragma unroll
        for (int c = 0; c < NC; ++c) logits_hi[(static_cast<size_t>(b) * NC + c) * pl_hi + static_cast<size_t>(oy) * W + ox] = v[c];
      }
      if (!labels) continue;
      const long long lab = labels[i];
      const size_t pl_hi2 = static_cast<size_t>(H) * W;
      float* d = dlogit_hi + static_cast<size_t>(b) * NC * pl_hi2 + static_cast<size_t>(oy) * W + ox;
      if (lab == ignore) {
#pragma unroll
        for (int c = 0; c < NC; ++c) d[c * pl_hi2] = 0.f;
      } else {
        float s = 0.f;
#pragma unroll
        for (int c = 0; c < NC; ++c) { v[c] = __expf(v[c] - mx); s += v[c]; }
        const float inv = 1.f / s, invn = 1.f / static_cast<float>(n_valid[b]);
#pragma unroll
        for (int c = 0; c < NC; ++c) d[c * pl_hi2] = (v[c] * inv - (c == lab ? 1.f : 0.f)) * invn;
        lsum = -__logf(v[lab < NC && lab >= 0 ? lab : 0] * inv) * invn;
      }
    }
    if (loss) {
      const int b0 = __shfl_sync(0xffffffffu, b, 0);
      if (__all_sync(0xffffffffu, b == b0)) {
        float t = lsum;
#pragma unroll
        for (int o = 16; o > 0; o >>= 1) t += __shfl_xor_sync(0xffffffffu, t, o);
        if ((threadIdx.x & 31) == 0 && t != 0.f) atomicAdd(loss + b0, t);
      } else if (lsum != 0.f) {
        atomicAdd(loss + b, lsum);
      }
    }
  }
}

template <int NC>
__global__ void logits_bilinear_bwd_kernel(const float* __restrict__ dhi, __nv_bfloat16* __restrict__ dlo, int B, int h,
                                           int w, int H, int W, int CP, int ldo) {
  pdl_prologue();
  const size_t total = static_cast<size_t>(B) * h * w;
  const float sy = static_cast<float>(h) / H, sx = static_cast<float>(w) / W;
  const int fy = (H + h - 1) / h, fx = (W + w - 1) / w;
  for (size_t i = blockIdx.x * static_cast<size_t>(blockDim.x) + threadIdx.x; i < total;
       i += static_cast<size_t>(gridDim.x) * blockDim.x) {
    const int ix = static_cast<int>(i % w), iy = static_cast<int>((i / w) % h), b = static_cast<int>(i / (static_cast<size_t>(w) * h));
    float acc[NC];
#pragma unroll
    for (int c = 0; c < NC; ++c) acc[c] = 0.f;
    const int oy_lo = max(0, fy * iy - fy - 1), oy_hi = min(H - 1, fy * iy + 2 * fy);
    const int ox_lo = max(0, fx * ix - fx - 1), ox_hi = min(W - 1, fx * ix + 2 * fx);
    for (int oy = oy_lo; oy <= oy_hi; ++oy) {
      int y0, y1; float ly;
      bilinear_src(oy, sy, h, y0, y1, ly);
      float wy = 0.f;
      if (y0 == iy) wy += 1.f - ly;
      if (y1 == iy) wy += ly;
      if (wy == 0.f) continue;
      for (int ox = ox_lo; ox <= ox_hi; ++ox) {
        int x0, x1; float lx;
        bilinear_src(ox, sx, w, x0, x1, lx);
        float wx = 0.f;
        if (x0 == ix) wx += 1.f - lx;
        if (x1 == ix) wx += lx;
        if (wx == 0.f) continue;
        const float ww = wy * wx;
        const size_t plane = static_cast<size_t>(H) * W;
        const float* d = dhi + static_cast<size_t>(b) * NC * plane + static_cast<size_t>(oy) * W + ox;
#pragma unroll
        for (int c = 0; c < NC; ++c) acc[c] += ww * __ldg(d + c * plane);
      }
    }
    __nv_bfloat16* o = dlo + i * ldo;
    for (int c = 0; c < CP; ++c) o[c] = __float2bfloat16_rn(c < NC ? acc[c] : 0.f);
  }
}

constexpr int kLhTY = 4, kLhTX = 8, kLhThreads = 256;
template <int NC>
__global__ void __launch_bounds__(kLhThreads)
seg_loss_head_fused_kernel(const float* __restrict__ logits_lo, const long long* __restrict__ labels, const int* __restrict__ n_valid,
                           long long* __restrict__ pred, float* __restrict__ loss, __nv_bfloat16* __restrict__ dlo, int h, int w,
                           int H, int W, int fy, int fx, int RWmax, int CP, int ldo, int ignore) {
  pdl_prologue();
  extern __shared__ float lh_s[];
  __shared__ float lh_loss[kLhThreads / 32];
  const int b = blockIdx.z, ty0 = blockIdx.y * kLhTY, tx0 = blockIdx.x * kLhTX;
  const float sy = static_cast<float>(h) / H, sx = static_cast<float>(w) / W;
  const int ry0 = max(0, fy * ty0 - (fy + 1) / 2), ry1 = min(H - 1, fy * (ty0 + kLhTY - 1) + (3 * fy) / 2);
  const int rx0 = max(0, fx * tx0 - (fx + 1) / 2), rx1 = min(W - 1, fx * (tx0 + kLhTX - 1) + (3 * fx) / 2);
  const int RH = ry1 - ry0 + 1, RW = rx1 - rx0 + 1;
  (void)RWmax;
  const size_t plane = static_cast<size_t>(h) * w, plane_hi = static_cast<size_t>(H) * W;
  const float* lb = logits_lo + static_cast<size_t>(b) * NC * plane;
  const float invn = 1.f / static_cast<float>(max(n_valid[b], 1));
  float lsum = 0.f;
  for (int idx = threadIdx.x; idx < RH * RW; idx += kLhThreads) {
    const int oy = ry0 + idx / RW, ox = rx0 + idx % RW;
    int y0, y1, x0, x1;
    float ly, lx;
    bilinear_src(oy, sy, h, y0, y1, ly);
    bilinear_src(ox, sx, w, x0, x1, lx);
    const float w00 = (1.f - ly) * (1.f - lx), w01 = (1.f - ly) * lx, w10 = ly * (1.f - lx), w11 = ly * lx;
    float v[NC];
    float mx = -INFINITY;
    int am = 0;
#pragma unroll
    for (int c = 0; c < NC; ++c) {
      const float* pl = lb + c * plane;
      v[c] = w00 * __ldg(pl + y0 * w + x0) + w01 * __ldg(pl + y0 * w + x1) + w10 * __ldg(pl + y1 * w + x0) + w11 * __ldg(pl + y1 * w + x1);
      if (v[c] > mx) { mx = v[c]; am = c; }
    }
    const size_t hi = static_cast<size_t>(b) * plane_hi + static_cast<size_t>(oy) * W + ox;
    const long long lab = labels[hi];
    const bool owned = (oy / fy >= ty0) && (oy / fy < ty0 + kLhTY) && (ox / fx >= tx0) && (ox / fx < tx0 + kLhTX);
    if (owned && pred) pred[hi] = am;
    float* d = lh_s + static_cast<size_t>(idx) * NC;
    if (lab == ignore) {
#pragma unroll
      for (int c = 0; c < NC; ++c) d[c] = 0.f;
    } else {
      float s = 0.f;
#pragma unroll
      for (int c = 0; c < NC; ++c) { v[c] = __expf(v[c] - mx); s += v[c]; }
      const float inv = 1.f / s;
#pragma unroll
      for (int c = 0; c < NC; ++c) d[c] = (v[c] * inv - (c == lab ? 1.f : 0.f)) * invn;
      if (owned) lsum -= __logf(v[lab < NC && lab >= 0 ? lab : 0] * inv) * invn;
    }
  }
  if (loss) {
#pragma unroll
    for (int o = 16; o > 0; o >>= 1) lsum += __shfl_xor_sync(0xffffffffu, lsum, o);
    if ((threadIdx.x & 31) == 0) lh_loss[threadIdx.x >> 5] = lsum;
  }
  __syncthreads();
  if (loss && threadIdx.x == 0) {
    float t = 0.f;
#pragma unroll
    for (int i = 0; i < kLhThreads / 32; ++i) t += lh_loss[i];
    if (t != 0.f) atomicAdd(loss + b, t);
  }
  const int p = threadIdx.x >> 3, k = threadIdx.x & 7;
  const int iy = ty0 + p / kLhTX, ix = tx0 + p % kLhTX;
  if (iy >= h || ix >= w) return;
  float acc[3] = {0.f, 0.f, 0.f};
  constexpr int kMaxTap = 16;
  float wys[kMaxTap], wxs[kMaxTap];
  int nyt = 0, nxt = 0, oy_first = 0, ox_first = 0;
  {
    const int lo = max(ry0, fy * iy - (fy + 1) / 2), hi = min(ry1, fy * iy + (3 * fy) / 2);
    oy_first = lo;
    for (int oy = lo; oy <= hi && nyt < kMaxTap; ++oy) {
      int y0, y1; float ly;
      bilinear_src(oy, sy, h, y0, y1, ly);
      float wy = 0.f;
      if (y0 == iy) wy += 1.f - ly;
      if (y1 == iy) wy += ly;
      wys[nyt++] = wy;
    }
  }
  {
    const int lo = max(rx0, fx * ix - (fx + 1) / 2), hi = min(rx1, fx * ix + (3 * fx) / 2);
    ox_first = lo;
    for (int ox = lo; ox <= hi && nxt < kMaxTap; ++ox) {
      int x0, x1; float lx;
      bilinear_src(ox, sx, w, x0, x1, lx);
      float wx = 0.f;
      if (x0 == ix) wx += 1.f - lx;
      if (x1 == ix) wx += lx;
      wxs[nxt++] = wx;
    }
  }
#pragma unroll 1
  for (int jy = 0; jy < nyt; ++jy) {
    const float wy = wys[jy];
    if (wy == 0.f) continue;
    const float* drow = lh_s + (static_cast<size_t>(oy_first + jy - ry0) * RW + (ox_first - rx0)) * NC + k;
#pragma unroll 4
    for (int jx = 0; jx < nxt; ++jx) {
      const float ww = wy * wxs[jx];
      const float* d = drow + jx * NC;
      acc[0] += ww * d[0];
      acc[1] += ww * d[8];
      if (k + 16 < NC) acc[2] += ww * d[16];
    }
  }
  __nv_bfloat16* o = dlo + ((static_cast<size_t>(b) * h + iy) * w + ix) * ldo;
  for (int c = k, j = 0; c < CP; c += 8, ++j) o[c] = __float2bfloat16_rn(c < NC ? acc[j] : 0.f);
}

__global__ void __launch_bounds__(128)
conv1_dgrad_kernel(const __nv_bfloat16* __restrict__ dz, const float* __restrict__ w ,
                   const float* __restrict__ scale, float* __restrict__ dx, int B, int H, int W, int Ho, int Wo) {
  pdl_prologue();
  extern __shared__ float sw[];
  for (int i = threadIdx.x; i < 49 * 3 * 64; i += blockDim.x) {
    const int o = i & 63, c = (i >> 6) % 3, t = i / 192;
    sw[i] = w[(static_cast<size_t>(o) * 3 + c) * 49 + t] * (scale ? scale[o] : 1.f);
  }
  __syncthreads();
  const int py = blockIdx.y >> 1, px = blockIdx.y & 1;
  const int Hh = H / 2, Wh = W / 2;
  const size_t total = static_cast<size_t>(B) * Hh * Wh;
  for (size_t i = blockIdx.x * static_cast<size_t>(blockDim.x) + threadIdx.x; i < total;
       i += static_cast<size_t>(gridDim.x) * blockDim.x) {
    const int xh = static_cast<int>(i % Wh), yh = static_cast<int>((i / Wh) % Hh), b = static_cast<int>(i / (static_cast<size_t>(Wh) * Hh));
    const int x = 2 * xh + px, y = 2 * yh + py;
    float2 a0 = make_float2(0.f, 0.f), a1 = a0, a2 = a0;
    for (int ky = (py + 1) & 1; ky < 7; ky += 2) {
      const int ny = y + 3 - ky;
      const int oy = ny >> 1;
      if (ny < 0 || oy >= Ho) continue;
      for (int kx = (px + 1) & 1; kx < 7; kx += 2) {
        const int nx = x + 3 - kx;
        const int ox = nx >> 1;
        if (nx < 0 || ox >= Wo) continue;
        const uint4* zp = reinterpret_cast<const uint4*>(dz + ((static_cast<size_t>(b) * Ho + oy) * Wo + ox) * 64);
        const float4* wp = reinterpret_cast<const float4*>(sw + (ky * 7 + kx) * 192);
#pragma unroll
        for (int o8 = 0; o8 < 8; ++o8) {
          const uint4 u = __ldg(zp + o8);
          const float2 f0 = unpack_bf16(u.x), f1 = unpack_bf16(u.y), f2 = unpack_bf16(u.z), f3 = unpack_bf16(u.w);
          const float4 w0a = wp[o8 * 2], w0b = wp[o8 * 2 + 1];
          const float4 w1a = wp[16 + o8 * 2], w1b = wp[16 + o8 * 2 + 1];
          const float4 w2a = wp[32 + o8 * 2], w2b = wp[32 + o8 * 2 + 1];
          a0 = ffma2(f0, make_float2(w0a.x, w0a.y), a0); a0 = ffma2(f1, make_float2(w0a.z, w0a.w), a0);
          a0 = ffma2(f2, make_float2(w0b.x, w0b.y), a0); a0 = ffma2(f3, make_float2(w0b.z, w0b.w), a0);
          a1 = ffma2(f0, make_float2(w1a.x, w1a.y), a1); a1 = ffma2(f1, make_float2(w1a.z, w1a.w), a1);
          a1 = ffma2(f2, make_float2(w1b.x, w1b.y), a1); a1 = ffma2(f3, make_float2(w1b.z, w1b.w), a1);
          a2 = ffma2(f0, make_float2(w2a.x, w2a.y), a2); a2 = ffma2(f1, make_float2(w2a.z, w2a.w), a2);
          a2 = ffma2(f2, make_float2(w2b.x, w2b.y), a2); a2 = ffma2(f3, make_float2(w2b.z, w2b.w), a2);
        }
      }
    }
    const size_t plane = static_cast<size_t>(H) * W, o = static_cast<size_t>(b) * 3 * plane + static_cast<size_t>(y) * W + x;
    dx[o] = a0.x + a0.y; dx[o + plane] = a1.x + a1.y; dx[o + 2 * plane] = a2.x + a2.y;
  }
}

__global__ void conv1_dgrad_weff_kernel(const float* __restrict__ w, const float* __restrict__ scale, float* __restrict__ weff,
                                        int P) {
  pdl_prologue();
  const int R = P / 2 + 3;
  const int total = R * R * 3 * 64;
  for (int idx = blockIdx.x * blockDim.x + threadIdx.x; idx < total; idx += gridDim.x * blockDim.x) {
    const int o = idx & 63, c = (idx >> 6) % 3, rs = idx / 192, s_ = rs % R - 1, r_ = rs / R - 1;
    float acc = 0.f;
    for (int j = 0; j < P; ++j) {
      const int ky = j + 3 - 2 * r_;
      if (ky < 0 || ky > 6) continue;
      for (int i = 0; i < P; ++i) {
        const int kx = i + 3 - 2 * s_;
        if (kx < 0 || kx > 6) continue;
        acc += w[((static_cast<size_t>(o) * 3 + c) * 7 + ky) * 7 + kx];
      }
    }
    weff[idx] = acc * (scale ? scale[o] : 1.f) / static_cast<float>(P * P);
  }
}

__global__ void __launch_bounds__(128)
conv1_dgrad_pooled_kernel(const __nv_bfloat16* __restrict__ dz, const float* __restrict__ weff, float* __restrict__ out, int B,
                          int Ho, int Wo, int P) {
  pdl_prologue();
  extern __shared__ float sw[];
  const int R = P / 2 + 3, half = P / 2;
  for (int i = threadIdx.x; i < R * R * 192; i += blockDim.x) sw[i] = weff[i];
  __syncthreads();
  const int Hp = Ho / half, Wp = Wo / half;
  const size_t total = static_cast<size_t>(B) * Hp * Wp;
  for (size_t i = blockIdx.x * static_cast<size_t>(blockDim.x) + threadIdx.x; i < total;
       i += static_cast<size_t>(gridDim.x) * blockDim.x) {
    const int X = static_cast<int>(i % Wp), Y = static_cast<int>((i / Wp) % Hp), b = static_cast<int>(i / (static_cast<size_t>(Wp) * Hp));
    float2 a0 = make_float2(0.f, 0.f), a1 = a0, a2 = a0;
    for (int r = 0; r < R; ++r) {
      const int oy = half * Y + r - 1;
      if (oy < 0 || oy >= Ho) continue;
      for (int s_ = 0; s_ < R; ++s_) {
        const int ox = half * X + s_ - 1;
        if (ox < 0 || ox >= Wo) continue;
        const uint4* zp = reinterpret_cast<const uint4*>(dz + ((static_cast<size_t>(b) * Ho + oy) * Wo + ox) * 64);
        const float4* wp = reinterpret_cast<const float4*>(sw + (r * R + s_) * 192);
#pragma unroll
        for (int o8 = 0; o8 < 8; ++o8) {
          const uint4 u = __ldg(zp + o8);
          const float2 f0 = unpack_bf16(u.x), f1 = unpack_bf16(u.y), f2 = unpack_bf16(u.z), f3 = unpack_bf16(u.w);
          const float4 w0a = wp[o8 * 2], w0b = wp[o8 * 2 + 1];
          const float4 w1a = wp[16 + o8 * 2], w1b = wp[16 + o8 * 2 + 1];
          const float4 w2a = wp[32 + o8 * 2], w2b = wp[32 + o8 * 2 + 1];
          a0 = ffma2(f0, make_float2(w0a.x, w0a.y), a0); a0 = ffma2(f1, make_float2(w0a.z, w0a.w), a0);
          a0 = ffma2(f2, make_float2(w0b.x, w0b.y), a0); a0 = ffma2(f3, make_float2(w0b.z, w0b.w), a0);
          a1 = ffma2(f0, make_float2(w1a.x, w1a.y), a1); a1 = ffma2(f1, make_float2(w1a.z, w1a.w), a1);
          a1 = ffma2(f2, make_float2(w1b.x, w1b.y), a1); a1 = ffma2(f3, make_float2(w1b.z, w1b.w), a1);
          a2 = ffma2(f0, make_float2(w2a.x, w2a.y), a2); a2 = ffma2(f1, make_float2(w2a.z, w2a.w), a2);
          a2 = ffma2(f2, make_float2(w2b.x, w2b.y), a2); a2 = ffma2(f3, make_float2(w2b.z, w2b.w), a2);
        }
      }
    }
    const size_t plane = static_cast<size_t>(Hp) * Wp, o = static_cast<size_t>(b) * 3 * plane + static_cast<size_t>(Y) * Wp + X;
    out[o] = a0.x + a0.y; out[o + plane] = a1.x + a1.y; out[o + 2 * plane] = a2.x + a2.y;
  }
}

__global__ void relu_mask_kernel(__nv_bfloat16* __restrict__ d, const __nv_bfloat16* __restrict__ m, size_t npix, int C,
                                 int ldd, int ldm) {
  pdl_prologue();
  const size_t total = npix * C;
  for (size_t i = blockIdx.x * static_cast<size_t>(blockDim.x) + threadIdx.x; i < total;
       i += static_cast<size_t>(gridDim.x) * blockDim.x) {
    const size_t p = i / C;
    const int c = static_cast<int>(i % C);
    if (!(__bfloat162float(m[p * ldm + c]) > 0.f)) d[p * ldd + c] = __float2bfloat16_rn(0.f);
  }
}

__global__ void compose_sep_kernel(const float* __restrict__ dw, const float* __restrict__ pw, const float* __restrict__ dwb,
                                   const float* __restrict__ pwb, float* __restrict__ w, float* __restrict__ bias, int Co,
                                   int Ci, int KK) {
  pdl_prologue();
  const size_t total = static_cast<size_t>(Co) * Ci * KK;
  for (size_t i = blockIdx.x * static_cast<size_t>(blockDim.x) + threadIdx.x; i < total;
       i += static_cast<size_t>(gridDim.x) * blockDim.x) {
    const int t = static_cast<int>(i % KK), c = static_cast<int>((i / KK) % Ci), o = static_cast<int>(i / (static_cast<size_t>(KK) * Ci));
    w[i] = pw[static_cast<size_t>(o) * Ci + c] * dw[static_cast<size_t>(c) * KK + t];
  }
  if (bias) {
    for (int o = blockIdx.x * blockDim.x + threadIdx.x; o < Co; o += gridDim.x * blockDim.x) {
      float s = pwb ? pwb[o] : 0.f;
      if (dwb)
        for (int c = 0; c < Ci; ++c) s += pw[static_cast<size_t>(o) * Ci + c] * dwb[c];
      bias[o] = s;
    }
  }
}

}

int bn_fold(const float* g, const float* b, const float* mean, const float* var, float eps, float* scale, float* shift,
            int n, int n_pad, cudaStream_t st) {
  launch_k(bn_fold_kernel, (n_pad + 255) / 256, 256, 0, st, g, b, mean, var, eps, scale, shift, n, n_pad);
  WC_LAUNCH_CHECK();
  return 0;
}
int maxpool_fwd(const __nv_bfloat16* x, __nv_bfloat16* y, uint8_t* idx, int B, int H, int W, int C, cudaStream_t st) {
  const int Ho = (H + 2 - 3) / 2 + 1, Wo = (W + 2 - 3) / 2 + 1;
  ProfScope prof(kProfOther, st, 0);
  launch_k(maxpool_fwd_kernel, grid_for(static_cast<size_t>(B) * Ho * Wo * C / 8), 256, 0, st, x, y, idx, B, H, W, C, Ho, Wo);
  WC_LAUNCH_CHECK();
  return 0;
}
int maxpool_bwd(const __nv_bfloat16* dy, const uint8_t* idx, const __nv_bfloat16* x, __nv_bfloat16* dx, int B, int H,
                int W, int C, cudaStream_t st) {
  const int Ho = (H + 2 - 3) / 2 + 1, Wo = (W + 2 - 3) / 2 + 1;
  ProfScope prof(kProfOther, st, 0);
  launch_k(maxpool_bwd_kernel, grid_for(static_cast<size_t>(B) * H * W * C / 8), 256, 0, st, dy, idx, x, dx, B, H, W, C, Ho, Wo);
  WC_LAUNCH_CHECK();
  return 0;
}
int gap_fwd(const __nv_bfloat16* x, __nv_bfloat16* y, int B, int HW, int C, int ld, cudaStream_t st) {
  ProfScope prof(kProfOther, st, 0);
  launch_k(gap_fwd_kernel, dim3((C + 63) / 64, B), 256, 0, st, x, y, HW, C, ld);
  WC_LAUNCH_CHECK();
  return 0;
}
int broadcast_hw(const __nv_bfloat16* v, __nv_bfloat16* y, int B, int HW, int C, int ldy, cudaStream_t st) {
  ProfScope prof(kProfOther, st, 0);
  launch_k(broadcast_kernel, grid_for(static_cast<size_t>(B) * HW * C / 8), 256, 0, st, v, y, B, HW, C, ldy);
  WC_LAUNCH_CHECK();
  return 0;
}
int sum_hw(const __nv_bfloat16* y, const __nv_bfloat16* mask, __nv_bfloat16* v, int B, int HW, int C, int ldy, cudaStream_t st) {
  ProfScope prof(kProfOther, st, 0);
  launch_k(sum_hw_kernel, dim3((C + 63) / 64, B), 256, 0, st, y, mask, v, HW, C, ldy);
  WC_LAUNCH_CHECK();
  return 0;
}
int gap_bwd_add(const __nv_bfloat16* g, __nv_bfloat16* dx, int B, int HW, int C, int ld, cudaStream_t st) {
  ProfScope prof(kProfOther, st, 0);
  launch_k(gap_bwd_add_kernel, grid_for(static_cast<size_t>(B) * HW * C), 256, 0, st, g, dx, B, HW, C, ld);
  WC_LAUNCH_CHECK();
  return 0;
}
int bilinear_fwd(const __nv_bfloat16* x, __nv_bfloat16* y, int B, int Hi, int Wi, int Ho, int Wo, int C, int ldx, int ldy,
                 cudaStream_t st) {
  WC_REQUIRE(C % 8 == 0, "bilinear: C must be a multiple of 8");
  ProfScope prof(kProfOther, st, 0);
  launch_k(bilinear_fwd_kernel, grid_for(static_cast<size_t>(B) * Ho * Wo * C / 8), 256, 0, st, x, y, B, Hi, Wi, Ho, Wo, C, ldx, ldy);
  WC_LAUNCH_CHECK();
  return 0;
}
int bilinear_bwd(const __nv_bfloat16* dy, const __nv_bfloat16* mask, __nv_bfloat16* dx, int B, int Hi, int Wi, int Ho,
                 int Wo, int C, int ldy, int ldm, int ldx, cudaStream_t st) {
  ProfScope prof(kProfOther, st, 0);
  WC_REQUIRE(C % 8 == 0 && ldy % 8 == 0 && ldx % 8 == 0, "bilinear_bwd: channels / strides must be multiples of 8");
  launch_k(bilinear_bwd_kernel, grid_for(static_cast<size_t>(B) * Hi * Wi * C / 8), 256, 0, st, dy, mask, dx, B, Hi, Wi, Ho, Wo, C, ldy, ldm, ldx);
  WC_LAUNCH_CHECK();
  return 0;
}
int seg_loss_grad(const float* logits_lo, const long long* labels, int* n_valid, long long* pred, float* dlogit_hi,
                  float* loss, float* logits_hi, int B, int h, int w, int H, int W, int nc, int ignore, cudaStream_t st) {
  WC_REQUIRE(nc == 19, "loss head is compiled for 19 classes (Cityscapes trainIds)");
  WC_REQUIRE(labels || (!pred && !dlogit_hi && !loss), "seg_loss_grad without labels writes the up-sampled logits only");
  ProfScope prof(kProfOther, st, 0);
  if (labels) {
    WC_CHECK_CUDA(cudaMemsetAsync(n_valid, 0, B * sizeof(int), st));
    if (loss) WC_CHECK_CUDA(cudaMemsetAsync(loss, 0, B * sizeof(float), st));
    launch_k(count_valid_kernel, dim3(std::min(64, (H * W + 255) / 256), B), 256, 0, st, labels, H * W, ignore, n_valid);
    WC_LAUNCH_CHECK();
  }
  launch_k(seg_loss_grad_kernel<19>, grid_for(static_cast<size_t>(B) * H * W, 128), 128, 0, st, logits_lo, labels, n_valid, pred, dlogit_hi, loss, logits_hi, B, h, w, H, W, ignore);
  WC_LAUNCH_CHECK();
  return 0;
}
int seg_loss_head_fused(const float* logits_lo, const long long* labels, int* n_valid, long long* pred, float* loss,
                        __nv_bfloat16* dlo, int B, int h, int w, int H, int W, int nc, int cp, int ldo, int ignore, cudaStream_t st) {
  WC_REQUIRE(nc == 19, "loss head is compiled for 19 classes (Cityscapes trainIds)");
  if (H % h != 0 || W % w != 0 || cp > 32) return -1;
  const int fy = H / h, fx = W / w;
  if (fy > 8 || fx > 8) return -1;
  const int RH = fy * (kLhTY - 1) + (3 * fy) / 2 + (fy + 1) / 2 + 1, RW = fx * (kLhTX - 1) + (3 * fx) / 2 + (fx + 1) / 2 + 1;
  const size_t smem = static_cast<size_t>(RH) * RW * 19 * sizeof(float) + 64;
  if (smem > 200 * 1024) return -1;
  static size_t attr = 0;
  if (smem > attr) {
    WC_CHECK_CUDA(cudaFuncSetAttribute(seg_loss_head_fused_kernel<19>, cudaFuncAttributeMaxDynamicSharedMemorySize, static_cast<int>(smem)));
    attr = smem;
  }
  ProfScope prof(kProfOther, st, 0);
  WC_CHECK_CUDA(cudaMemsetAsync(n_valid, 0, B * sizeof(int), st));
  if (loss) WC_CHECK_CUDA(cudaMemsetAsync(loss, 0, B * sizeof(float), st));
  launch_k(count_valid_kernel, dim3(std::min(64, (H * W + 255) / 256), B), 256, 0, st, labels, H * W, ignore, n_valid);
  WC_LAUNCH_CHECK();
  launch_k(seg_loss_head_fused_kernel<19>, dim3((w + kLhTX - 1) / kLhTX, (h + kLhTY - 1) / kLhTY, B), kLhThreads, smem, st, logits_lo, labels,
           n_valid, pred, loss, dlo, h, w, H, W, fy, fx, RW, cp, ldo, ignore);
  WC_LAUNCH_CHECK();
  return 0;
}
int logits_bilinear_bwd(const float* dhi, __nv_bfloat16* dlo, int B, int h, int w, int H, int W, int nc, int cp, int ldo,
                        cudaStream_t st) {
  WC_REQUIRE(nc == 19, "loss head is compiled for 19 classes");
  ProfScope prof(kProfOther, st, 0);
  launch_k(logits_bilinear_bwd_kernel<19>, grid_for(static_cast<size_t>(B) * h * w, 128), 128, 0, st, dhi, dlo, B, h, w, H, W, cp, ldo);
  WC_LAUNCH_CHECK();
  return 0;
}
int conv1_dgrad(const __nv_bfloat16* dz, const float* w, const float* scale, float* dx, int B, int H, int W, int Cout,
                cudaStream_t st) {
  WC_REQUIRE(Cout == 64 && H % 2 == 0 && W % 2 == 0, "conv1 data gradient is built for 64 output channels and even image dims");
  const int Ho = H / 2, Wo = W / 2;
  const size_t smem = static_cast<size_t>(49) * 64 * 3 * sizeof(float);
  ProfScope prof(kProfBoundaryConv, st, static_cast<double>(B) * (12.0 * H * W + 2.0 * Ho * Wo * Cout));
  const int gx = std::max(1, grid_for(static_cast<size_t>(B) * Ho * Wo, 128) / 2);
  launch_k(conv1_dgrad_kernel, dim3(gx, 4), 128, smem, st, dz, w, scale, dx, B, H, W, Ho, Wo);
  WC_LAUNCH_CHECK();
  return 0;
}
int conv1_dgrad_weff(const float* w, const float* scale, float* weff, int P, cudaStream_t st) {
  launch_k(conv1_dgrad_weff_kernel, 8, 256, 0, st, w, scale, weff, P);
  WC_LAUNCH_CHECK();
  return 0;
}
int conv1_dgrad_pooled(const __nv_bfloat16* dz, const float* weff, float* out, int B, int H, int W, int P, cudaStream_t st) {
  WC_REQUIRE(P >= 2 && P % 2 == 0 && P <= 8 && H % P == 0 && W % P == 0, "pooled stem gradient needs an even pool <= 8 dividing H and W");
  const int R = P / 2 + 3;
  const size_t smem = static_cast<size_t>(R) * R * 192 * sizeof(float);
  static size_t attr = 0;
  if (smem > 48 * 1024 && smem > attr) {
    WC_CHECK_CUDA(cudaFuncSetAttribute(conv1_dgrad_pooled_kernel, cudaFuncAttributeMaxDynamicSharedMemorySize, static_cast<int>(smem)));
    attr = smem;
  }
  ProfScope prof(kProfBoundaryConv, st, static_cast<double>(B) * (12.0 * (H / P) * (W / P) + 2.0 * (H / 2) * (W / 2) * 64));
  launch_k(conv1_dgrad_pooled_kernel, grid_for(static_cast<size_t>(B) * (H / P) * (W / P), 128), 128, smem, st, dz, weff, out, B, H / 2, W / 2, P);
  WC_LAUNCH_CHECK();
  return 0;
}
int relu_mask_inplace(__nv_bfloat16* d, const __nv_bfloat16* m, size_t npix, int C, int ldd, int ldm, cudaStream_t st) {
  ProfScope prof(kProfOther, st, 0);
  launch_k(relu_mask_kernel, grid_for(npix * C), 256, 0, st, d, m, npix, C, ldd, ldm);
  WC_LAUNCH_CHECK();
  return 0;
}
int compose_sep(const float* dw, const float* pw, const float* dwb, const float* pwb, float* w, float* bias, int Co, int Ci,
                int KK, cudaStream_t st) {
  launch_k(compose_sep_kernel, grid_for(static_cast<size_t>(Co) * Ci * KK), 256, 0, st, dw, pw, dwb, pwb, w, bias, Co, Ci, KK);
  WC_LAUNCH_CHECK();
  return 0;
}

}

namespace wc {
namespace {

constexpr int kFT_H = 8, kFT_W = 64, kFHalo = 4, kFPlaneW = kFT_W + 2 * kFHalo , kFPlaneH = kFT_H + 2 * kFHalo ;
constexpr int kFPlane = kFPlaneW * kFPlaneH + 1;

template <bool HALF>
__global__ void __launch_bounds__(512, 1)
srgan_final_kernel(const __nv_bfloat16* __restrict__ x, const float* __restrict__ dw ,
                   const float* __restrict__ dwb, const float* __restrict__ pw , const float* __restrict__ pwb,
                   float* __restrict__ y, int B, int H, int W, int ldx) {
  pdl_prologue();
  extern __shared__ uint32_t sm[];
  uint32_t* tile = sm;
  float* wsm = reinterpret_cast<float*>(sm + 32 * kFPlane);
  float* red = wsm + 32 * 81 * 2;
  const int tiles_x = (W + kFT_W - 1) / kFT_W, tiles_y = (H + kFT_H - 1) / kFT_H;
  const int tid = threadIdx.x;
  if (HALF) {
    __half2* wh = reinterpret_cast<__half2*>(wsm);
    for (int i = tid; i < 32 * 81; i += 512) {
      const int tap = i % 81, c2 = i / 81;
      wh[i] = __floats2half2_rn(dw[(c2 * 2) * 81 + tap], dw[(c2 * 2 + 1) * 81 + tap]);
    }
  } else {
    for (int i = tid; i < 32 * 81 * 2; i += 512) {
      const int j = i & 1, tap = (i >> 1) % 81, c2 = (i >> 1) / 81;
      wsm[i] = dw[(c2 * 2 + j) * 81 + tap];
    }
  }
  const int grp = tid >> 7, t = tid & 127, tx = t & 63, ty = (t >> 6) * 4;
  for (int tl = blockIdx.x; tl < B * tiles_x * tiles_y; tl += gridDim.x) {
    const int b = tl / (tiles_x * tiles_y), r = tl % (tiles_x * tiles_y), y0 = (r / tiles_x) * kFT_H, x0 = (r % tiles_x) * kFT_W;
    __syncthreads();
    for (int i = tid; i < kFPlaneH * kFPlaneW * 8; i += 512) {
      const int c8 = i & 7, px = (i >> 3) % kFPlaneW, py = (i >> 3) / kFPlaneW;
      const int gy = y0 + py - kFHalo, gx = x0 + px - kFHalo;
      uint4 u = make_uint4(0, 0, 0, 0);
      if (gy >= 0 && gy < H && gx >= 0 && gx < W)
        u = __ldg(reinterpret_cast<const uint4*>(x + ((static_cast<size_t>(b) * H + gy) * W + gx) * ldx + c8 * 8));
      uint32_t* dst = tile + (c8 * 4) * kFPlane + py * kFPlaneW + px;
      if (HALF) {
        auto h2 = [](uint32_t w) {
          const __half2 h = __floats2half2_rn(__uint_as_float(w << 16), __uint_as_float(w & 0xffff0000u));
          return *reinterpret_cast<const uint32_t*>(&h);
        };
        u.x = h2(u.x); u.y = h2(u.y); u.z = h2(u.z); u.w = h2(u.w);
      }
      dst[0] = u.x; dst[kFPlane] = u.y; dst[2 * kFPlane] = u.z; dst[3 * kFPlane] = u.w;
    }
    __syncthreads();
    float o[3][4];
#pragma unroll
    for (int n = 0; n < 3; ++n)
#pragma unroll
      for (int p = 0; p < 4; ++p) o[n][p] = 0.f;
    for (int c2 = grp * 8; c2 < grp * 8 + 8; ++c2) {
      float2 acc2[4];
      const float b0 = dwb ? dwb[2 * c2] : 0.f, b1 = dwb ? dwb[2 * c2 + 1] : 0.f;
#pragma unroll
      for (int p = 0; p < 4; ++p) acc2[p] = make_float2(b0, b1);
      const uint32_t* pl = tile + c2 * kFPlane + ty * kFPlaneW + tx;
      const float2* wp = reinterpret_cast<const float2*>(wsm) + c2 * 81;
      if (HALF) {
        const __half2* wh = reinterpret_cast<const __half2*>(wsm) + c2 * 81;
#pragma unroll
        for (int kx = 0; kx < 9; ++kx) {
          __half2 v[12];
#pragma unroll
          for (int i = 0; i < 12; ++i) {
            const uint32_t u = pl[i * kFPlaneW + kx];
            v[i] = *reinterpret_cast<const __half2*>(&u);
          }
          __half2 part[4];
#pragma unroll
          for (int p = 0; p < 4; ++p) part[p] = __hmul2(v[p], wh[kx]);
#pragma unroll
          for (int ky = 1; ky < 9; ++ky) {
            const __half2 wv = wh[ky * 9 + kx];
#pragma unroll
            for (int p = 0; p < 4; ++p) part[p] = __hfma2(v[p + ky], wv, part[p]);
          }
#pragma unroll
          for (int p = 0; p < 4; ++p) {
            const float2 f = __half22float2(part[p]);
            acc2[p].x += f.x; acc2[p].y += f.y;
          }
        }
      } else
#pragma unroll
      for (int kx = 0; kx < 9; ++kx) {
        float2 v[12];
#pragma unroll
        for (int i = 0; i < 12; ++i) {
          const uint32_t u = pl[i * kFPlaneW + kx];
          v[i] = make_float2(__uint_as_float(u << 16), __uint_as_float(u & 0xffff0000u));
        }
#pragma unroll
        for (int ky = 0; ky < 9; ++ky) {
          const float2 wv = wp[ky * 9 + kx];
#pragma unroll
          for (int p = 0; p < 4; ++p) acc2[p] = ffma2(v[p + ky], wv, acc2[p]);
        }
      }
#pragma unroll
      for (int n = 0; n < 3; ++n) {
        const float w0 = pw[n * 64 + 2 * c2], w1 = pw[n * 64 + 2 * c2 + 1];
#pragma unroll
        for (int p = 0; p < 4; ++p) o[n][p] = fmaf(acc2[p].x, w0, fmaf(acc2[p].y, w1, o[n][p]));
      }
    }
    if (grp > 0) {
#pragma unroll
      for (int n = 0; n < 3; ++n)
#pragma unroll
        for (int p = 0; p < 4; ++p) red[((grp - 1) * 128 + t) * 12 + n * 4 + p] = o[n][p];
    }
    __syncthreads();
    if (grp == 0) {
      const int gx = x0 + tx;
      const size_t plane = static_cast<size_t>(H) * W;
#pragma unroll
      for (int n = 0; n < 3; ++n)
#pragma unroll
        for (int p = 0; p < 4; ++p) {
          const int gy = y0 + ty + p;
          if (gy < H && gx < W) {
            const float v = o[n][p] + red[t * 12 + n * 4 + p] + red[(128 + t) * 12 + n * 4 + p] + red[(256 + t) * 12 + n * 4 + p] +
                            (pwb ? pwb[n] : 0.f);
            y[(static_cast<size_t>(b) * 3 + n) * plane + static_cast<size_t>(gy) * W + gx] = (tanhf(v) + 1.f) * 0.5f;
          }
        }
    }
  }
}

__global__ void srgan_final_compose_kernel(const float* __restrict__ dw, const float* __restrict__ dwb, const float* __restrict__ pw,
                                           const float* __restrict__ pwb, float* __restrict__ wq ,
                                           float* __restrict__ bias3) {
  pdl_prologue();
  const int i = blockIdx.x * blockDim.x + threadIdx.x;
  if (i < 32 * 64 * 9) {
    const int tx = i % 9, c = (i / 9) % 64, n = i / (9 * 64);
    float v = 0.f;
    if (n < 27) {
      const int ty = n / 3, o = n % 3;
      v = pw[o * 64 + c] * dw[(c * 9 + ty) * 9 + tx];
    }
    wq[i] = v;
  }
  if (i < 3) {
    float b = pwb ? pwb[i] : 0.f;
    if (dwb)
      for (int c = 0; c < 64; ++c) b = fmaf(pw[i * 64 + c], dwb[c], b);
    bias3[i] = b;
  }
}

__global__ void __launch_bounds__(256)
srgan_final_combine_kernel(const float* __restrict__ t , const float* __restrict__ bias3, float* __restrict__ y ,
                           int H, int W4) {
  pdl_prologue();
  const int x4 = blockIdx.x * blockDim.x + threadIdx.x;
  const int yy = blockIdx.y, b = blockIdx.z;
  if (x4 >= W4) return;
  const size_t plane4 = static_cast<size_t>(H) * W4;
  const float4* tp = reinterpret_cast<const float4*>(t) + static_cast<size_t>(b) * 27 * plane4 + x4;
  float4 acc[3];
#pragma unroll
  for (int o = 0; o < 3; ++o) {
    const float bo = bias3[o];
    acc[o] = make_float4(bo, bo, bo, bo);
  }
#pragma unroll
  for (int ty = 0; ty < 9; ++ty) {
    const int r = yy + ty - 4;
    if (r < 0 || r >= H) continue;
#pragma unroll
    for (int o = 0; o < 3; ++o) {
      const float4 v = __ldg(tp + static_cast<size_t>(ty * 3 + o) * plane4 + static_cast<size_t>(r) * W4);
      acc[o].x += v.x; acc[o].y += v.y; acc[o].z += v.z; acc[o].w += v.w;
    }
  }
  float4* yp = reinterpret_cast<float4*>(y) + static_cast<size_t>(b) * 3 * plane4 + static_cast<size_t>(yy) * W4 + x4;
#pragma unroll
  for (int o = 0; o < 3; ++o) {
    float4 v;
    v.x = (tanhf(acc[o].x) + 1.f) * 0.5f; v.y = (tanhf(acc[o].y) + 1.f) * 0.5f;
    v.z = (tanhf(acc[o].z) + 1.f) * 0.5f; v.w = (tanhf(acc[o].w) + 1.f) * 0.5f;
    yp[static_cast<size_t>(o) * plane4] = v;
  }
}

__global__ void phase_major_rows_kernel(const float* __restrict__ src, float* __restrict__ dst, int cb, int len, int rep_src) {
  pdl_prologue();
  const size_t i = blockIdx.x * static_cast<size_t>(blockDim.x) + threadIdx.x;
  if (i >= static_cast<size_t>(4) * cb * len) return;
  const int e = static_cast<int>(i % len), n = static_cast<int>(i / len), q = n / cb, c = n % cb;
  dst[i] = src[static_cast<size_t>(rep_src ? c : c * 4 + q) * len + e];
}

__global__ void gather_stride_kernel(const float* src, float* dst, int n, int mul, int off) {
  pdl_prologue();
  const int i = blockIdx.x * blockDim.x + threadIdx.x;
  if (i < n) dst[i] = src[i * mul + off];
}

}

int srgan_final(const __nv_bfloat16* x, const float* dw, const float* dwb, const float* pw, const float* pwb, float* y, int B,
                int H, int W, int ldx, cudaStream_t st) {
  const size_t smem = (32 * kFPlane) * 4 + 32 * 81 * 2 * 4 + 3 * 128 * 12 * 4;
  static bool attr = false;
  if (!attr) {
    WC_CHECK_CUDA(cudaFuncSetAttribute(srgan_final_kernel<false>, cudaFuncAttributeMaxDynamicSharedMemorySize, static_cast<int>(smem)));
    WC_CHECK_CUDA(cudaFuncSetAttribute(srgan_final_kernel<true>, cudaFuncAttributeMaxDynamicSharedMemorySize, static_cast<int>(smem)));
    attr = true;
  }
  static int half = -1;
  if (half < 0) {
    const char* e = getenv("WC_SRGAN_FINAL_F16");
    half = e ? atoi(e) : 1;
  }
  const int tiles = B * ((W + kFT_W - 1) / kFT_W) * ((H + kFT_H - 1) / kFT_H);
  ProfScope prof(kProfBoundaryConv, st, static_cast<double>(B) * H * W * (128.0 + 12.0));
  if (half) launch_k(srgan_final_kernel<true>, std::min(tiles, num_sms()), 512, smem, st, x, dw, dwb, pw, pwb, y, B, H, W, ldx);
  else launch_k(srgan_final_kernel<false>, std::min(tiles, num_sms()), 512, smem, st, x, dw, dwb, pw, pwb, y, B, H, W, ldx);
  WC_LAUNCH_CHECK();
  return 0;
}
int srgan_final_compose(const float* dw, const float* dwb, const float* pw, const float* pwb, float* wq, float* bias3, cudaStream_t st) {
  launch_k(srgan_final_compose_kernel, (32 * 64 * 9 + 255) / 256, 256, 0, st, dw, dwb, pw, pwb, wq, bias3);
  WC_LAUNCH_CHECK();
  return 0;
}
int srgan_final_combine(const float* t, const float* bias3, float* y, int B, int H, int W, cudaStream_t st) {
  WC_REQUIRE(W % 4 == 0, "srgan_final_combine: width must be a multiple of 4");
  const int W4 = W / 4;
  ProfScope prof(kProfBoundaryConv, st, static_cast<double>(B) * H * W * (27.0 * 4 + 12.0));
  launch_k(srgan_final_combine_kernel, dim3((W4 + 255) / 256, H, B), 256, 0, st, t, bias3, y, H, W4);
  WC_LAUNCH_CHECK();
  return 0;
}
constexpr int kSI_T = 16;
__global__ void __launch_bounds__(kSI_T * kSI_T)
srgan_initial_kernel(const float* __restrict__ x, const float* __restrict__ dw, const float* __restrict__ dwb,
                     const float* __restrict__ pw, const float* __restrict__ pwb, const float* __restrict__ slope,
                     __nv_bfloat16* __restrict__ y, int H, int W, int ldy) {
  pdl_prologue();
  constexpr int HT = kSI_T + 8;
  __shared__ float tile[3][HT][HT + 1];
  __shared__ float s_dw[3][81], s_pw[64][3], s_b[64], s_sl[64], s_dwb[3];
  const int tid = threadIdx.y * kSI_T + threadIdx.x;
  const int b = blockIdx.z, x0 = blockIdx.x * kSI_T, y0 = blockIdx.y * kSI_T;
  for (int i = tid; i < 243; i += kSI_T * kSI_T) s_dw[i / 81][i % 81] = dw[i];
  for (int i = tid; i < 192; i += kSI_T * kSI_T) s_pw[i / 3][i % 3] = pw[i];
  if (tid < 64) { s_b[tid] = pwb ? pwb[tid] : 0.f; s_sl[tid] = slope[tid]; }
  if (tid < 3) s_dwb[tid] = dwb ? dwb[tid] : 0.f;
  const float* xb = x + static_cast<size_t>(b) * 3 * H * W;
  for (int i = tid; i < 3 * HT * HT; i += kSI_T * kSI_T) {
    const int c = i / (HT * HT), r = (i / HT) % HT, q = i % HT;
    const int yy = y0 + r - 4, xx = x0 + q - 4;
    tile[c][r][q] = (yy >= 0 && yy < H && xx >= 0 && xx < W) ? xb[(static_cast<size_t>(c) * H + yy) * W + xx] : 0.f;
  }
  __syncthreads();
  const int px = x0 + threadIdx.x, py = y0 + threadIdx.y;
  if (px >= W || py >= H) return;
  float d[3];
#pragma unroll
  for (int c = 0; c < 3; ++c) {
    float a = s_dwb[c];
#pragma unroll
    for (int ky = 0; ky < 9; ++ky)
#pragma unroll
      for (int kx = 0; kx < 9; ++kx) a = fmaf(tile[c][threadIdx.y + ky][threadIdx.x + kx], s_dw[c][ky * 9 + kx], a);
    d[c] = a;
  }
  uint4* dst = reinterpret_cast<uint4*>(y + ((static_cast<size_t>(b) * H + py) * W + px) * ldy);
#pragma unroll
  for (int j = 0; j < 8; ++j) {
    float v[8];
#pragma unroll
    for (int i = 0; i < 8; ++i) {
      const int n = 8 * j + i;
      float a = fmaf(d[2], s_pw[n][2], fmaf(d[1], s_pw[n][1], fmaf(d[0], s_pw[n][0], s_b[n])));
      v[i] = a > 0.f ? a : a * s_sl[n];
    }
    uint4 u;
    u.x = pack_bf16(v[0], v[1]); u.y = pack_bf16(v[2], v[3]); u.z = pack_bf16(v[4], v[5]); u.w = pack_bf16(v[6], v[7]);
    dst[j] = u;
  }
}

int srgan_initial(const float* x, const float* dw, const float* dwb, const float* pw, const float* pwb, const float* slope,
                  __nv_bfloat16* y, int B, int H, int W, int ldy, cudaStream_t st) {
  WC_REQUIRE(ldy % 8 == 0, "output pixel stride must be a multiple of 8");
  ProfScope prof(kProfBoundaryConv, st, static_cast<double>(B) * H * W * (3 * 4.0 + 64 * 2.0));
  dim3 grid((W + kSI_T - 1) / kSI_T, (H + kSI_T - 1) / kSI_T, B);
  launch_k(srgan_initial_kernel, grid, dim3(kSI_T, kSI_T), 0, st, x, dw, dwb, pw, pwb, slope, y, H, W, ldy);
  WC_LAUNCH_CHECK();
  return 0;
}

int phase_major_rows(const float* src, float* dst, int cb, int len, int rep_src, cudaStream_t st) {
  const size_t total = static_cast<size_t>(4) * cb * len;
  launch_k(phase_major_rows_kernel, static_cast<int>((total + 255) / 256), 256, 0, st, src, dst, cb, len, rep_src);
  WC_LAUNCH_CHECK();
  return 0;
}
int gather_stride(const float* src, float* dst, int n, int mul, int off, cudaStream_t st) {
  launch_k(gather_stride_kernel, (n + 255) / 256, 256, 0, st, src, dst, n, mul, off);
  WC_LAUNCH_CHECK();
  return 0;
}
}

namespace wc {
namespace {

__global__ void srgan_tanh_bwd_kernel(const float* __restrict__ dy, const float* __restrict__ y, float* __restrict__ dz, size_t n) {
  pdl_prologue();
  for (size_t i = blockIdx.x * static_cast<size_t>(blockDim.x) + threadIdx.x; i < n; i += static_cast<size_t>(gridDim.x) * blockDim.x) {
    const float v = y[i];
    dz[i] = dy[i] * (2.f * v * (1.f - v));
  }
}

__global__ void flip_transpose_kk_kernel(const float* __restrict__ w, float* __restrict__ wt, int Co, int Ci, int KK) {
  pdl_prologue();
  const int i = blockIdx.x * blockDim.x + threadIdx.x;
  if (i >= Co * Ci * KK) return;
  const int t = i % KK, ci = (i / KK) % Ci, co = i / (KK * Ci);
  wt[(static_cast<size_t>(ci) * Co + co) * KK + (KK - 1 - t)] = w[i];
}

__global__ void prelu_bwd_kernel(__nv_bfloat16* __restrict__ d, const __nv_bfloat16* __restrict__ add,
                                 const __nv_bfloat16* __restrict__ pre, const float* __restrict__ slope, size_t npix, int C, int ldd,
                                 int lda, int ldp) {
  pdl_prologue();
  const int c8n = C / 8;
  for (size_t i = blockIdx.x * static_cast<size_t>(blockDim.x) + threadIdx.x; i < npix * c8n; i += static_cast<size_t>(gridDim.x) * blockDim.x) {
    const size_t p = i / c8n;
    const int c0 = static_cast<int>(i % c8n) * 8;
    uint4* dp = reinterpret_cast<uint4*>(d + p * ldd + c0);
    const uint4 u = *dp, m = *reinterpret_cast<const uint4*>(pre + p * ldp + c0);
    const uint4 a = add ? *reinterpret_cast<const uint4*>(add + p * lda + c0) : make_uint4(0, 0, 0, 0);
    const uint32_t uu[4] = {u.x, u.y, u.z, u.w}, mm[4] = {m.x, m.y, m.z, m.w}, aa[4] = {a.x, a.y, a.z, a.w};
    uint32_t o[4];
#pragma unroll
    for (int k = 0; k < 4; ++k) {
      const float2 g = unpack_bf16(uu[k]), s = unpack_bf16(mm[k]), q = unpack_bf16(aa[k]);
      const float gx = g.x + q.x, gy = g.y + q.y;
      o[k] = pack_bf16(s.x > 0.f ? gx : gx * slope[c0 + 2 * k], s.y > 0.f ? gy : gy * slope[c0 + 2 * k + 1]);
    }
    *dp = make_uint4(o[0], o[1], o[2], o[3]);
  }
}

__global__ void shuffle_prelu_bwd_kernel(const __nv_bfloat16* __restrict__ dup, const __nv_bfloat16* __restrict__ pre,
                                         const float* __restrict__ slope, __nv_bfloat16* __restrict__ dconv, int B, int h, int w, int C) {
  pdl_prologue();
  const int k8 = C / 2;
  const size_t total = static_cast<size_t>(B) * h * w * k8;
  for (size_t i = blockIdx.x * static_cast<size_t>(blockDim.x) + threadIdx.x; i < total; i += static_cast<size_t>(gridDim.x) * blockDim.x) {
    const int k = static_cast<int>(i % k8);
    const size_t pix = i / k8;
    const int x = static_cast<int>(pix % w), y = static_cast<int>((pix / w) % h), b = static_cast<int>(pix / (static_cast<size_t>(w) * h));
    const int c = 2 * k;
    const float s0 = slope[c], s1 = slope[c + 1];
    float v[8];
#pragma unroll
    for (int q = 0; q < 4; ++q) {
      const size_t off = ((static_cast<size_t>(b) * 2 * h + 2 * y + (q >> 1)) * 2 * w + 2 * x + (q & 1)) * C + c;
      const float2 g = unpack_bf16(*reinterpret_cast<const uint32_t*>(dup + off));
      const float2 m = unpack_bf16(*reinterpret_cast<const uint32_t*>(pre + off));
      v[q] = m.x > 0.f ? g.x : g.x * s0;
      v[4 + q] = m.y > 0.f ? g.y : g.y * s1;
    }
    uint4 o;
    o.x = pack_bf16(v[0], v[1]); o.y = pack_bf16(v[2], v[3]); o.z = pack_bf16(v[4], v[5]); o.w = pack_bf16(v[6], v[7]);
    *reinterpret_cast<uint4*>(dconv + pix * (4 * C) + 8 * k) = o;
  }
}

__global__ void fill_f32_kernel(float* __restrict__ p, float v, int n) {
  pdl_prologue();
  const int i = blockIdx.x * blockDim.x + threadIdx.x;
  if (i < n) p[i] = v;
}

}

int srgan_tanh_bwd(const float* dy, const float* y, float* dz, size_t n, cudaStream_t st) {
  ProfScope prof(kProfOther, st, 0);
  launch_k(srgan_tanh_bwd_kernel, grid_for(n), 256, 0, st, dy, y, dz, n);
  WC_LAUNCH_CHECK();
  return 0;
}
int flip_transpose_kk(const float* w, float* wt, int Co, int Ci, int KK, cudaStream_t st) {
  launch_k(flip_transpose_kk_kernel, (Co * Ci * KK + 255) / 256, 256, 0, st, w, wt, Co, Ci, KK);
  WC_LAUNCH_CHECK();
  return 0;
}
int prelu_bwd(__nv_bfloat16* d, const __nv_bfloat16* add, const __nv_bfloat16* pre, const float* slope, size_t npix, int C, int ldd,
              int lda, int ldp, cudaStream_t st) {
  WC_REQUIRE(C % 8 == 0 && ldd % 8 == 0 && lda % 8 == 0 && ldp % 8 == 0, "prelu_bwd: channels and pixel strides must be multiples of 8");
  ProfScope prof(kProfOther, st, 0);
  launch_k(prelu_bwd_kernel, grid_for(npix * (C / 8)), 256, 0, st, d, add, pre, slope, npix, C, ldd, lda, ldp);
  WC_LAUNCH_CHECK();
  return 0;
}
int shuffle_prelu_bwd(const __nv_bfloat16* dup, const __nv_bfloat16* pre, const float* slope, __nv_bfloat16* dconv, int B, int h, int w,
                      int C, cudaStream_t st) {
  WC_REQUIRE(C % 2 == 0, "shuffle_prelu_bwd: even channel count");
  ProfScope prof(kProfOther, st, 0);
  launch_k(shuffle_prelu_bwd_kernel, grid_for(static_cast<size_t>(B) * h * w * (C / 2)), 256, 0, st, dup, pre, slope, dconv, B, h, w, C);
  WC_LAUNCH_CHECK();
  return 0;
}
int fill_f32(float* p, float v, int n, cudaStream_t st) {
  launch_k(fill_f32_kernel, (n + 255) / 256, 256, 0, st, p, v, n);
  WC_LAUNCH_CHECK();
  return 0;
}
}
```

### weatherconverter_b200/csrc/wc_api.cu

```cuda
#include "../../include/wc_b200.h"

#include "conv.cuh"
#include "wgrad.cuh"

namespace wc {
int ddpm_step(const float* xt, const float* eps, const float* z, float* out, float* mean_out, float* sigz_out,
              size_t n_per_sample, int B, float beta, float s, float sqrt_alpha, float sigma, cudaStream_t st);
int ddpm_step_batched(const float* xt, const float* eps, const float* z, float* out, float* mean_out, float* sigz_out,
                      size_t n_per_sample, int B, const float* betas, const float* alphas, const float* sqrt_1m_acp,
                      const long long* t, int T, cudaStream_t st);
int ddpm_step_indexed(const float* xt, const float* eps, const float* z, float* out, float* mean_out, float* sigz_out,
                      size_t n_per_sample, int B, const float* coef_tables, const long long* t_dev, int T, cudaStream_t st);
int ddim_step(const float* xt, const float* eps, const float* z, float* out, float* mean_out, float* sigz_out,
              size_t n_per_sample, int B, float a_t, float s_t, float a_prev, float d, float sigma, cudaStream_t st);
int ddim_step_indexed(const float* xt, const float* eps, const float* z, float* out, float* mean_out, float* sigz_out,
                      size_t n_per_sample, int B, const float* coef_tables, const long long* t_dev, int T, cudaStream_t st);
int add_noise(const float* x0, const float* noise, float* out, size_t n_per_sample, int B, const float* sqrt_acp,
              const float* sqrt_1m_acp, const long long* t, int T, cudaStream_t st);
int sgg_update(const float* grad, const float* mu, const float* sigz, float* out, float* mag_out, int B, int h, int w,
               int pool, float lam, cudaStream_t st);
int lcg_prepare(const float* sr, const long long* gt, float* xm, long long* gm, int B, int NC, size_t hw, cudaStream_t st);
int lcg_combine(const float* g4, const long long* gt, const float* mu, const float* sigz, float* out, int B, int NC, int h,
                int w, int pool, float lam, cudaStream_t st);
int groupnorm_silu(const __nv_bfloat16* x, __nv_bfloat16* y, int B, int HW, int C, int ld, int ldy, const float* gamma,
                   const float* beta, float eps, int silu, void* workspace, cudaStream_t st);
size_t groupnorm_workspace_bytes(int B);
int conv_small_cin(const float* x, const float* w, const float* bias, const float* scale, const float* shift,
                   __nv_bfloat16* y, int B, int Cin, int H, int W, int Cout, int K, int stride, int pad, int ldy,
                   int relu, cudaStream_t st, const float* prelu = nullptr);
int conv_small_cout(const __nv_bfloat16* x, const float* w, const float* bias, float* y, int B, int H, int W, int Cin,
                    int Cout, int K, int ldx, int tanh_out, cudaStream_t st);
int nchw_f32_to_nhwc_bf16(const float* x, __nv_bfloat16* y, int B, int C, int HW, int ldy, cudaStream_t st);
int nhwc_bf16_to_nchw_f32(const __nv_bfloat16* x, float* y, int B, int C, int HW, int ldx, cudaStream_t st);
void prof_start();
int prof_detail(int cap, int* cls, double* ms, double* work, int* info);
int prof_stop(double* ms, long long* count, double* work);
int attention_forward(const __nv_bfloat16* q, const __nv_bfloat16* k, const __nv_bfloat16* vt, __nv_bfloat16* out, int B,
                      int heads, int ntok, int hd, int ldo, cudaStream_t st, float* lse = nullptr, float scale = 0.f);
int maxpool_fwd(const __nv_bfloat16* x, __nv_bfloat16* y, uint8_t* idx, int B, int H, int W, int C, cudaStream_t st);
int maxpool_bwd(const __nv_bfloat16* dy, const uint8_t* idx, const __nv_bfloat16* x, __nv_bfloat16* dx, int B, int H,
                int W, int C, cudaStream_t st);
int bilinear_fwd(const __nv_bfloat16* x, __nv_bfloat16* y, int B, int Hi, int Wi, int Ho, int Wo, int C, int ldx, int ldy,
                 cudaStream_t st);
int bilinear_bwd(const __nv_bfloat16* dy, const __nv_bfloat16* mask, __nv_bfloat16* dx, int B, int Hi, int Wi, int Ho,
                 int Wo, int C, int ldy, int ldm, int ldx, cudaStream_t st);
int seg_loss_grad(const float* logits_lo, const long long* labels, int* n_valid, long long* pred, float* dlogit_hi,
                  float* loss, float* logits_hi, int B, int h, int w, int H, int W, int nc, int ignore, cudaStream_t st);
int seg_loss_head_fused(const float* logits_lo, const long long* labels, int* n_valid, long long* pred, float* loss,
                        __nv_bfloat16* dlo, int B, int h, int w, int H, int W, int nc, int cp, int ldo, int ignore, cudaStream_t st);
int logits_bilinear_bwd(const float* dhi, __nv_bfloat16* dlo, int B, int h, int w, int H, int W, int nc, int cp, int ldo,
                        cudaStream_t st);
int conv1_dgrad(const __nv_bfloat16* dz, const float* w, const float* scale, float* dx, int B, int H, int W, int Cout,
                cudaStream_t st);
int groupnorm_silu_bwd(const __nv_bfloat16* x, const __nv_bfloat16* dy, __nv_bfloat16* dx, int B, int HW, int C, int ld,
                       int ldd, int ldo, const float* gamma, const float* beta, float eps, int silu, const void* stats,
                       const __nv_bfloat16* add1, int lda1, const __nv_bfloat16* add2, int lda2, float* dgamma, float* dbeta,
                       void* workspace, cudaStream_t st);
size_t groupnorm_bwd_workspace_bytes(int B, int Cmax);
int colsum(const __nv_bfloat16* x, int B, int HW, int C, int ld, float* out_rows, int ldo, float* out_total, void* workspace,
           cudaStream_t st);
int attention_backward(const __nv_bfloat16* q, const __nv_bfloat16* k, const __nv_bfloat16* v, const __nv_bfloat16* d_o, int ldd,
                       const float* lse, const float* D, __nv_bfloat16* dqkv, int ld3, int B, int heads, int ntok, int hd,
                       cudaStream_t st);
int attn_rowdot(const __nv_bfloat16* o, const __nv_bfloat16* d_o, int ldo, int ldd, int B, int ntok, int heads, int hd, float* D,
                cudaStream_t st);
int mse_loss_grad(const float* pred, const float* target, float* dpred, size_t n, float grad_scale, float* loss, void* scratch,
                  cudaStream_t st);
size_t boundary_wgrad_scratch_bytes();
int boundary_wgrad(const __nv_bfloat16* wide, int ldw, const float* narrow, int B, int H, int W, int sign, float* dw,
                   float* dbias, void* scratch, cudaStream_t st);
int adam_step(float* p, const float* g, float* m, float* v, size_t n, float lr, float beta1, float beta2, float eps, int step,
              float grad_scale, cudaStream_t st);
int time_embedding(const long long* t, int n, int dim, float* out, cudaStream_t st);
int ddpm_grid_u8(const float* x, uint8_t* out, int B, int H, int W, int nrow, int pad, cudaStream_t st);
int postprocess_u8(const float* x, uint8_t* out, int B, int H, int W, const float* mean3, const float* std3, cudaStream_t st);
int label_encode(const uint8_t* lab, int Ws, const int* ytab, const int* xtab, int top, int left, int Hc, int Wc, const long long* lut,
                 int nlut, long long* out, cudaStream_t st);
int resample_u8(const uint8_t* in, uint8_t* tmp, uint8_t* out, int Hin, int Win, int Hout, int Wout, int C, const int* bounds_h,
                const int* kk_h, int ksize_h, const int* bounds_v, const int* kk_v, int ksize_v, cudaStream_t st);
int u8_to_tensor(const uint8_t* in, int Win, int top, int left, int Hc, int Wc, int mode, const float* mean3, const float* std3, float* out,
                 cudaStream_t st);
}

using namespace wc;
static inline cudaStream_t S(void* s) { return static_cast<cudaStream_t>(s); }
static inline __nv_bfloat16* BF(wc_bf16* p) { return reinterpret_cast<__nv_bfloat16*>(p); }
static inline const __nv_bfloat16* BF(const wc_bf16* p) { return reinterpret_cast<const __nv_bfloat16*>(p); }

extern "C" {

const char* wc_last_error(void) { return last_error_cstr(); }
int wc_abi_version(void) { return 6; }
long long wc_launch_count(void) { return launch_count(); }
void wc_profile_begin(void) { prof_start(); }
int wc_profile_detail(int cap, int* cls, double* ms, double* work, int* info) { return prof_detail(cap, cls, ms, work, info); }
int wc_profile_end(double* ms_by_class, long long* count_by_class, double* work_by_class) {
  return prof_stop(ms_by_class, count_by_class, work_by_class);
}

int wc_ddpm_step(const float* xt, const float* eps, const float* z, float* out, float* mean_out, float* sigz_out,
                 size_t n_per_sample, int batch, float beta, float sqrt_one_minus_acp, float sqrt_alpha, float sigma,
                 void* stream) {
  return ddpm_step(xt, eps, z, out, mean_out, sigz_out, n_per_sample, batch, beta, sqrt_one_minus_acp, sqrt_alpha, sigma,
                   S(stream));
}
int wc_ddpm_step_batched(const float* xt, const float* eps, const float* z, float* out, float* mean_out,
                         float* sigz_out, size_t n_per_sample, int batch, const float* betas, const float* alphas,
                         const float* sqrt_one_minus_acp, const int64_t* t, int num_timesteps, void* stream) {
  return ddpm_step_batched(xt, eps, z, out, mean_out, sigz_out, n_per_sample, batch, betas, alphas, sqrt_one_minus_acp,
                           reinterpret_cast<const long long*>(t), num_timesteps, S(stream));
}
int wc_ddpm_step_indexed(const float* xt, const float* eps, const float* z, float* out, float* mean_out, float* sigz_out,
                         size_t n_per_sample, int batch, const float* coef_tables, const int64_t* t_dev, int num_timesteps,
                         void* stream) {
  return ddpm_step_indexed(xt, eps, z, out, mean_out, sigz_out, n_per_sample, batch, coef_tables,
                           reinterpret_cast<const long long*>(t_dev), num_timesteps, S(stream));
}
int wc_ddim_step(const float* xt, const float* eps, const float* z, float* out, float* mean_out, float* sigz_out,
                 size_t n_per_sample, int batch, float a_t, float s_t, float a_prev, float d, float sigma, void* stream) {
  return ddim_step(xt, eps, z, out, mean_out, sigz_out, n_per_sample, batch, a_t, s_t, a_prev, d, sigma, S(stream));
}
int wc_ddim_step_indexed(const float* xt, const float* eps, const float* z, float* out, float* mean_out, float* sigz_out,
                         size_t n_per_sample, int batch, const float* coef_tables, const int64_t* t_dev, int num_timesteps,
                         void* stream) {
  return ddim_step_indexed(xt, eps, z, out, mean_out, sigz_out, n_per_sample, batch, coef_tables,
                           reinterpret_cast<const long long*>(t_dev), num_timesteps, S(stream));
}
int wc_add_noise(const float* x0, const float* noise, float* out, size_t n_per_sample, int batch,
                 const float* sqrt_acp, const float* sqrt_one_minus_acp, const int64_t* t, int num_timesteps, void* stream) {
  return add_noise(x0, noise, out, n_per_sample, batch, sqrt_acp, sqrt_one_minus_acp,
                   reinterpret_cast<const long long*>(t), num_timesteps, S(stream));
}
int wc_set_time_factor_table(const float* factor_host, int half) { return set_time_factor_table(factor_host, half); }
int wc_time_embedding(const int64_t* t, int n, int dim, float* out, void* stream) {
  return time_embedding(reinterpret_cast<const long long*>(t), n, dim, out, S(stream));
}
int wc_sgg_update(const float* grad, const float* mu, const float* sigz, float* out, float* mag_out, int batch, int h,
                  int w, int pool, float lambda, void* stream) {
  return sgg_update(grad, mu, sigz, out, mag_out, batch, h, w, pool, lambda, S(stream));
}
int wc_lcg_prepare(const float* sr_xt, const int64_t* gt, float* x_masked, int64_t* gt_masked, int batch, int num_classes,
                   int H, int W, void* stream) {
  return lcg_prepare(sr_xt, reinterpret_cast<const long long*>(gt), x_masked, reinterpret_cast<long long*>(gt_masked), batch,
                     num_classes, static_cast<size_t>(H) * W, S(stream));
}
int wc_lcg_combine(const float* pooled_grads, const int64_t* gt, const float* mu, const float* sigz, float* out, int batch,
                   int num_classes, int h, int w, int pool, float lambda, void* stream) {
  return lcg_combine(pooled_grads, reinterpret_cast<const long long*>(gt), mu, sigz, out, batch, num_classes, h, w, pool, lambda,
                     S(stream));
}
size_t wc_groupnorm_workspace_bytes(int batch) { return groupnorm_workspace_bytes(batch); }
int wc_groupnorm_silu(const wc_bf16* x, wc_bf16* y, int batch, int hw, int channels, int ldx, int ldy,
                      const float* gamma, const float* beta, float eps, int silu, void* workspace, void* stream) {
  return groupnorm_silu(BF(x), BF(y), batch, hw, channels, ldx, ldy, gamma, beta, eps, silu, workspace, S(stream));
}

int wc_conv2d(const wc_bf16* x, int batch, int H, int W, int Cin, int ldx, const float* weight, const float* bias,
              int Cout, int K, int stride, int pad, int dil, int transposed, const float* rowbias,
              const wc_bf16* residual, int ldr, const wc_bf16* x2, int Cin2, int ldx2, const float* weight2, int relu,
              wc_bf16* y, int ldy, void* stream) {
  cudaStream_t st = S(stream);
  DeviceArena arena;
  ConvOp op;
  Act xin; xin.ptr = const_cast<__nv_bfloat16*>(BF(x)); xin.B = batch; xin.H = H; xin.W = W; xin.C = Cin; xin.ld = ldx;
  const int Ho = transposed ? H * 2 : (stride == 2 ? H / 2 : H), Wo = transposed ? W * 2 : (stride == 2 ? W / 2 : W);
  Act yout; yout.ptr = BF(y); yout.B = batch; yout.H = Ho; yout.W = Wo; yout.C = Cout; yout.ld = ldy;
  Act res; res.ptr = const_cast<__nv_bfloat16*>(BF(residual)); res.B = batch; res.H = Ho; res.W = Wo; res.C = Cout; res.ld = ldr;
  Act x2a; x2a.ptr = const_cast<__nv_bfloat16*>(BF(x2)); x2a.B = batch; x2a.H = H; x2a.W = W; x2a.C = Cin2; x2a.ld = ldx2;
  Epilogue ep; ep.bias = bias; ep.rowbias = rowbias; ep.ldrb = Cout; ep.res = residual ? &res : nullptr; ep.relu = relu;
  OutSpec os; os.mode = kOutNHWC; os.out = yout;
  int e;
  if (transposed) {
    WC_REQUIRE(stride == 2, "transposed convolution supports stride 2");
    WeightSrc w; w.w = weight; w.d0 = Cin; w.d1 = Cout; w.KH = w.KW = K; w.transpose = 1;
    e = build_conv_transposed_s2(&op, &arena, xin, w, K, pad, Cout, ep, os, st);
  } else {
    WeightSrc w; w.w = weight; w.d0 = Cout; w.d1 = Cin; w.KH = w.KW = K;
    WeightSrc w2; w2.w = weight2; w2.d0 = Cout; w2.d1 = Cin2;
    ConvGeom g; g.K = K; g.stride = stride; g.pad = pad; g.dil = dil;
    e = build_conv(&op, &arena, xin, w, g, Cout, x2 ? &x2a : nullptr, x2 ? &w2 : nullptr, ep, os, st);
  }
  if (e) return e;
  if ((e = op.run(st))) return e;
  WC_CHECK_CUDA(cudaStreamSynchronize(st));
  return 0;
}

int wc_conv2d_dgrad(const wc_bf16* dz, int batch, int Ho, int Wo, int Cout, const float* weight, int Cin, int K, int stride,
                    int dil, const wc_bf16* residual, const wc_bf16* mask, wc_bf16* dx, void* stream) {
  cudaStream_t st = S(stream);
  DeviceArena arena;
  ConvOp op;
  const int H = Ho * stride, W = Wo * stride;
  Act g; g.ptr = const_cast<__nv_bfloat16*>(BF(dz)); g.B = batch; g.H = Ho; g.W = Wo; g.C = Cout; g.ld = Cout;
  Act out; out.ptr = BF(dx); out.B = batch; out.H = H; out.W = W; out.C = Cin; out.ld = Cin;
  Act res = out; res.ptr = const_cast<__nv_bfloat16*>(BF(residual));
  Act msk = out; msk.ptr = const_cast<__nv_bfloat16*>(BF(mask));
  WeightSrc w; w.w = weight; w.d0 = Cout; w.d1 = Cin; w.KH = w.KW = K; w.transpose = 1;
  Epilogue ep; ep.res = residual ? &res : nullptr; ep.mask = mask ? &msk : nullptr;
  OutSpec os; os.mode = kOutNHWC; os.out = out;
  int e;
  if (stride == 1) {
    w.flip = 1;
    ConvGeom gg; gg.K = K; gg.stride = 1; gg.dil = dil; gg.pad = dil * (K - 1) / 2;
    e = build_conv(&op, &arena, g, w, gg, Cin, nullptr, nullptr, ep, os, st);
  } else {
    if (!residual) WC_CHECK_CUDA(cudaMemsetAsync(out.ptr, 0, out.pixels() * Cin * 2, st));
    e = build_conv_transposed_s2(&op, &arena, g, w, K, K == 3 ? 1 : 0, Cin, ep, os, st);
  }
  if (e) return e;
  if ((e = op.run(st))) return e;
  WC_CHECK_CUDA(cudaStreamSynchronize(st));
  return 0;
}
int wc_maxpool3x3s2(const wc_bf16* x, wc_bf16* y, uint8_t* idx, int batch, int H, int W, int C, void* stream) {
  return maxpool_fwd(BF(x), BF(y), idx, batch, H, W, C, S(stream));
}
int wc_maxpool3x3s2_bwd(const wc_bf16* dy, const uint8_t* idx, const wc_bf16* x, wc_bf16* dx, int batch, int H, int W, int C,
                        void* stream) {
  return maxpool_bwd(BF(dy), idx, BF(x), BF(dx), batch, H, W, C, S(stream));
}
int wc_bilinear(const wc_bf16* x, wc_bf16* y, int batch, int Hi, int Wi, int Ho, int Wo, int C, void* stream) {
  return bilinear_fwd(BF(x), BF(y), batch, Hi, Wi, Ho, Wo, C, C, C, S(stream));
}
int wc_bilinear_bwd(const wc_bf16* dy, const wc_bf16* mask, wc_bf16* dx, int batch, int Hi, int Wi, int Ho, int Wo, int C,
                    void* stream) {
  return bilinear_bwd(BF(dy), BF(mask), BF(dx), batch, Hi, Wi, Ho, Wo, C, C, C, C, S(stream));
}
int wc_seg_loss_head(const float* logits_lo, const int64_t* labels, int* n_valid_ws, int64_t* pred, float* dlogit_hi,
                     float* loss, float* logits_hi, wc_bf16* dlogit_lo, int batch, int h, int w, int H, int W, void* stream) {
  if (!dlogit_hi) {
    WC_REQUIRE(dlogit_lo && !logits_hi, "wc_seg_loss_head without dlogit_hi needs dlogit_lo and no logits_hi");
    const int e = seg_loss_head_fused(logits_lo, reinterpret_cast<const long long*>(labels), n_valid_ws, reinterpret_cast<long long*>(pred), loss,
                                      BF(dlogit_lo), batch, h, w, H, W, 19, 32, 32, 255, S(stream));
    if (e == -1) return fail("wc_seg_loss_head: the fused path needs integer up-sampling factors; pass dlogit_hi for the two-pass path");
    return e;
  }
  if (int e = seg_loss_grad(logits_lo, reinterpret_cast<const long long*>(labels), n_valid_ws,
                            reinterpret_cast<long long*>(pred), dlogit_hi, loss, logits_hi, batch, h, w, H, W, 19, 255, S(stream)))
    return e;
  if (dlogit_lo) return logits_bilinear_bwd(dlogit_hi, BF(dlogit_lo), batch, h, w, H, W, 19, 32, 32, S(stream));
  return 0;
}
int wc_conv1_dgrad(const wc_bf16* dz, const float* weight, const float* scale, float* dx, int batch, int H, int W, void* stream) {
  return conv1_dgrad(BF(dz), weight, scale, dx, batch, H, W, 64, S(stream));
}
int wc_conv_in(const float* x, const float* weight, const float* bias, const float* scale, const float* shift,
               wc_bf16* y, int batch, int H, int W, int Cout, int K, int stride, int pad, int ldy, int relu,
               void* stream) {
  return conv_small_cin(x, weight, bias, scale, shift, BF(y), batch, 3, H, W, Cout, K, stride, pad, ldy, relu, S(stream));
}
int wc_conv_out(const wc_bf16* x, const float* weight, const float* bias, float* y, int batch, int H, int W, int Cin,
                int K, int ldx, int tanh_out, void* stream) {
  return conv_small_cout(BF(x), weight, bias, y, batch, H, W, Cin, 3, K, ldx, tanh_out, S(stream));
}
int wc_nchw_f32_to_nhwc_bf16(const float* x, wc_bf16* y, int batch, int C, int hw, int ldy, void* stream) {
  return nchw_f32_to_nhwc_bf16(x, BF(y), batch, C, hw, ldy, S(stream));
}
int wc_nhwc_bf16_to_nchw_f32(const wc_bf16* x, float* y, int batch, int C, int hw, int ldx, void* stream) {
  return nhwc_bf16_to_nchw_f32(BF(x), y, batch, C, hw, ldx, S(stream));
}
int wc_attention(const wc_bf16* q, const wc_bf16* k, const wc_bf16* vt, wc_bf16* out, int batch, int heads, int ntok,
                 int hd, int ldo, void* stream) {
  return attention_forward(BF(q), BF(k), BF(vt), BF(out), batch, heads, ntok, hd, ldo, S(stream));
}


int wc_attention_scaled(const wc_bf16* q, const wc_bf16* k, const wc_bf16* vt, wc_bf16* out, int batch, int heads, int ntok,
                        int hd, int ldo, float scale, void* stream) {
  return attention_forward(BF(q), BF(k), BF(vt), BF(out), batch, heads, ntok, hd, ldo, S(stream), nullptr, scale);
}

int wc_attention_lse(const wc_bf16* q, const wc_bf16* k, const wc_bf16* vt, wc_bf16* out, float* lse, int batch, int heads,
                     int ntok, int hd, int ldo, void* stream) {
  return attention_forward(BF(q), BF(k), BF(vt), BF(out), batch, heads, ntok, hd, ldo, S(stream), lse);
}

int wc_attention_bwd(const wc_bf16* q, const wc_bf16* k, const wc_bf16* v, const wc_bf16* o, const wc_bf16* d_o, const float* lse,
                     float* d_scratch, wc_bf16* dqkv, int batch, int heads, int ntok, int hd, void* stream) {
  const int C = heads * hd;
  if (int e = attn_rowdot(BF(o), BF(d_o), C, C, batch, ntok, heads, hd, d_scratch, S(stream))) return e;
  return attention_backward(BF(q), BF(k), BF(v), BF(d_o), C, lse, d_scratch, BF(dqkv), 3 * C, batch, heads, ntok, hd, S(stream));
}

int wc_conv2d_wgrad(const wc_bf16* x, const wc_bf16* dy, int batch, int H, int W, int Cin, int Cout, int K, int stride, int pad,
                    int dil, int transposed, const wc_bf16* x2, int Cin2, float* dw, float* dw2, void* stream) {
  cudaStream_t st = S(stream);
  DeviceArena arena;
  float* partial = static_cast<float*>(arena.alloc(kWgradPartialBytes));
  if (!partial) return 1;
  const int Ho = transposed ? H * 2 : H / stride, Wo = transposed ? W * 2 : W / stride;
  Act xa; xa.ptr = const_cast<__nv_bfloat16*>(BF(x)); xa.B = batch; xa.H = H; xa.W = W; xa.C = Cin; xa.ld = Cin;
  Act dya; dya.ptr = const_cast<__nv_bfloat16*>(BF(dy)); dya.B = batch; dya.H = Ho; dya.W = Wo; dya.C = Cout; dya.ld = Cout;
  Act x2a = xa; x2a.ptr = const_cast<__nv_bfloat16*>(BF(x2)); x2a.C = Cin2; x2a.ld = Cin2;
  WgradOp op;
  int e = transposed ? build_convT_wgrad(&op, xa, dya, K, pad, dw, partial)
                     : build_conv_wgrad(&op, xa, dya, K, stride, pad, dil, dw, x2 ? &x2a : nullptr, dw2, partial);
  if (e) return e;
  if ((e = op.run(st))) return e;
  WC_CHECK_CUDA(cudaStreamSynchronize(st));
  return 0;
}

size_t wc_groupnorm_bwd_workspace_bytes(int batch, int channels) { return groupnorm_bwd_workspace_bytes(batch, channels); }
int wc_groupnorm_silu_bwd(const wc_bf16* x, const wc_bf16* dy, wc_bf16* dx, int batch, int hw, int channels, const float* gamma,
                          const float* beta, float eps, int silu, const void* fwd_workspace, const wc_bf16* add1,
                          const wc_bf16* add2, float* dgamma, float* dbeta, void* workspace, void* stream) {
  return groupnorm_silu_bwd(BF(x), BF(dy), BF(dx), batch, hw, channels, channels, channels, channels, gamma, beta, eps, silu,
                            fwd_workspace, BF(add1), channels, BF(add2), channels, dgamma, dbeta, workspace, S(stream));
}
int wc_colsum(const wc_bf16* x, int batch, int hw, int channels, float* out_rows, float* out_total, void* workspace, void* stream) {
  return colsum(BF(x), batch, hw, channels, channels, out_rows, channels, out_total, workspace, S(stream));
}
int wc_mse_loss_grad(const float* pred, const float* target, float* dpred, size_t n, float grad_scale, float* loss, void* scratch,
                     void* stream) {
  return mse_loss_grad(pred, target, dpred, n, grad_scale, loss, scratch, S(stream));
}
size_t wc_boundary_wgrad_scratch_bytes(void) { return boundary_wgrad_scratch_bytes(); }
int wc_boundary_wgrad(const wc_bf16* wide, const float* narrow, int batch, int H, int W, int sign, float* dw, float* dbias,
                      void* scratch, void* stream) {
  return boundary_wgrad(BF(wide), 64, narrow, batch, H, W, sign, dw, dbias, scratch, S(stream));
}
int wc_adam_step(float* p, const float* g, float* m, float* v, size_t n, float lr, float beta1, float beta2, float eps, int step,
                 float grad_scale, void* stream) {
  return adam_step(p, g, m, v, n, lr, beta1, beta2, eps, step, grad_scale, S(stream));
}


int wc_ddpm_grid_u8(const float* x, uint8_t* out, int batch, int H, int W, int nrow, int padding, void* stream) {
  return ddpm_grid_u8(x, out, batch, H, W, nrow, padding, S(stream));
}
int wc_postprocess_u8(const float* x, uint8_t* out, int batch, int H, int W, const float* mean3_host, const float* std3_host, void* stream) {
  return postprocess_u8(x, out, batch, H, W, mean3_host, std3_host, S(stream));
}
int wc_label_encode(const uint8_t* label_ids, int Ws, const int* ytab, const int* xtab, int top, int left, int Hc, int Wc,
                    const int64_t* lut, int nlut, int64_t* out, void* stream) {
  return label_encode(label_ids, Ws, ytab, xtab, top, left, Hc, Wc, reinterpret_cast<const long long*>(lut), nlut,
                      reinterpret_cast<long long*>(out), S(stream));
}
int wc_resample_u8(const uint8_t* in, uint8_t* tmp, uint8_t* out, int Hin, int Win, int Hout, int Wout, int channels, const int* bounds_h,
                   const int* kk_h, int ksize_h, const int* bounds_v, const int* kk_v, int ksize_v, void* stream) {
  return resample_u8(in, tmp, out, Hin, Win, Hout, Wout, channels, bounds_h, kk_h, ksize_h, bounds_v, kk_v, ksize_v, S(stream));
}
int wc_u8_to_tensor(const uint8_t* in, int Win, int top, int left, int Hc, int Wc, int mode, const float* mean3_host, const float* std3_host,
                    float* out, void* stream) {
  return u8_to_tensor(in, Win, top, left, Hc, Wc, mode, mean3_host, std3_host, out, S(stream));
}

}
```

Before: 2.980.

## Fuse maxpool backward into pooled stem dgrad with tensor-core MMA

Replaces the separate maxpool backward plus scalar pooled conv1 dgrad with one kernel. It rebuilds the pre-pool gradient tile in shared memory from the pool indices and ReLU mask, then runs the effective 3→64 conv through bf16 mma.sync. The effective weights are split into hi/lo bf16 pairs to keep precision. It also drops the standalone ReLU-mask and GAP-broadcast-add passes by folding them into the dgrad epilogue as a mask and row bias. This removes several full-tensor memory passes, at the cost of bf16 rounding of the recomputed gradient tile and more complex indexing.

```diff
diff --git a/include/wc_b200.h b/include/wc_b200.h
--- a/include/wc_b200.h
+++ b/include/wc_b200.h
@@ -69,6 +69,8 @@
 int wc_seg_loss_head(const float* logits_lo, const int64_t* labels, int* n_valid_ws, int64_t* pred, float* dlogit_hi,
                      float* loss, float* logits_hi, wc_bf16* dlogit_lo, int batch, int h, int w, int H, int W, void* stream);
 int wc_conv1_dgrad(const wc_bf16* dz, const float* weight, const float* scale, float* dx, int batch, int H, int W, void* stream);
+int wc_stem_bwd_pooled(const wc_bf16* gp, const uint8_t* idx, const wc_bf16* p1, const float* weight, const float* scale, float* out,
+                       int batch, int H, int W, int P, void* stream);
 int wc_nchw_f32_to_nhwc_bf16(const float* x, wc_bf16* y, int batch, int C, int hw, int ldy, void* stream);
 int wc_nhwc_bf16_to_nchw_f32(const wc_bf16* x, float* y, int batch, int C, int hw, int ldx, void* stream);
 int wc_attention(const wc_bf16* q, const wc_bf16* k, const wc_bf16* vt, wc_bf16* out, int batch, int heads, int ntok,
diff --git a/weatherconverter_b200/_lib.py b/weatherconverter_b200/_lib.py
--- a/weatherconverter_b200/_lib.py
+++ b/weatherconverter_b200/_lib.py
@@ -53,6 +53,7 @@
     "wc_bilinear_bwd": (C.c_int, [c_ptr] * 3 + [C.c_int] * 6 + [c_ptr]),
     "wc_seg_loss_head": (C.c_int, [c_ptr] * 8 + [C.c_int] * 5 + [c_ptr]),
     "wc_conv1_dgrad": (C.c_int, [c_ptr] * 4 + [C.c_int] * 3 + [c_ptr]),
+    "wc_stem_bwd_pooled": (C.c_int, [c_ptr] * 6 + [C.c_int] * 4 + [c_ptr]),
     "wc_conv_in": (C.c_int, [c_ptr] * 6 + [C.c_int] * 9 + [c_ptr]),
     "wc_conv_out": (C.c_int, [c_ptr] * 4 + [C.c_int] * 7 + [c_ptr]),
     "wc_nchw_f32_to_nhwc_bf16": (C.c_int, [c_ptr, c_ptr] + [C.c_int] * 4 + [c_ptr]),
diff --git a/weatherconverter_b200/csrc/seg.cu b/weatherconverter_b200/csrc/seg.cu
--- a/weatherconverter_b200/csrc/seg.cu
+++ b/weatherconverter_b200/csrc/seg.cu
@@ -13,7 +13,7 @@
 int gap_fwd(const __nv_bfloat16* x, __nv_bfloat16* y, int B, int HW, int C, int ld, cudaStream_t st);
 int broadcast_hw(const __nv_bfloat16* v, __nv_bfloat16* y, int B, int HW, int C, int ldy, cudaStream_t st);
 int sum_hw(const __nv_bfloat16* y, const __nv_bfloat16* mask, __nv_bfloat16* v, int B, int HW, int C, int ldy, cudaStream_t st);
-int gap_bwd_add(const __nv_bfloat16* g, __nv_bfloat16* dx, int B, int HW, int C, int ld, cudaStream_t st);
+int gap_bwd_rowbias(const __nv_bfloat16* g, float* rb, int B, int HW, int C, cudaStream_t st);
 int bilinear_fwd(const __nv_bfloat16* x, __nv_bfloat16* y, int B, int Hi, int Wi, int Ho, int Wo, int C, int ldx, int ldy,
                  cudaStream_t st);
 int bilinear_bwd(const __nv_bfloat16* dy, const __nv_bfloat16* mask, __nv_bfloat16* dx, int B, int Hi, int Wi, int Ho,
@@ -26,9 +26,10 @@
                         cudaStream_t st);
 int conv1_dgrad(const __nv_bfloat16* dz, const float* w, const float* scale, float* dx, int B, int H, int W, int Cout,
                 cudaStream_t st);
-int relu_mask_inplace(__nv_bfloat16* d, const __nv_bfloat16* m, size_t npix, int C, int ldd, int ldm, cudaStream_t st);
-int conv1_dgrad_weff(const float* w, const float* scale, float* weff, int P, cudaStream_t st);
-int conv1_dgrad_pooled(const __nv_bfloat16* dz, const float* weff, float* out, int B, int H, int W, int P, cudaStream_t st);
+size_t stem_bwd_frag_bytes(int P);
+int conv1_dgrad_weff(const float* w, const float* scale, __nv_bfloat16* frag, int P, cudaStream_t st);
+int stem_bwd_pooled(const __nv_bfloat16* gp, const uint8_t* idx, const __nv_bfloat16* p1, const __nv_bfloat16* frag, float* out, int B,
+                    int H, int W, int P, cudaStream_t st);
 }
 
 struct wc_seg {
@@ -113,12 +114,13 @@
   }
 
   void dgrad(const Act& dz, const std::string& wname, const std::string& bnname, int cin, int cout, int K, int stride,
-             int dil, const Act* res, const Act* mask, const Act& dx, const float* scale_override = nullptr, bool no_bn = false) {
+             int dil, const Act* res, const Act* mask, const Act& dx, const float* scale_override = nullptr, bool no_bn = false,
+             const float* rowbias = nullptr, int ldrb = 0) {
     if (dry) return;
     const float* sc = no_bn ? scale_override : bnfold(bnname, cout).first;
     WeightSrc w; w.w = P(wname + ".weight"); w.d0 = cout; w.d1 = cin; w.KH = w.KW = K; w.transpose = 1; w.scale = sc;
     if (err) return;
-    Epilogue ep; ep.res = res; ep.mask = mask;
+    Epilogue ep; ep.res = res; ep.mask = mask; ep.rowbias = rowbias; ep.ldrb = ldrb;
     OutSpec os; os.mode = kOutNHWC; os.out = dx;
     auto op = std::make_shared<ConvOp>();
     int e;
@@ -300,9 +302,8 @@
   Act dy = b.act(H4, W4, 256);
   b.dgrad(dlo19, c + ".classifier.3", "", 256, NC, 1, 1, 1, nullptr, &y, dy, nullptr, true);
   Act dcat2 = b.act(H4, W4, 304);
-  b.dgrad(dy, c + ".classifier.0", c + ".classifier.1", 304, 256, 3, 1, 1, nullptr, nullptr, dcat2);
+  b.dgrad(dy, c + ".classifier.0", c + ".classifier.1", 304, 256, 3, 1, 1, nullptr, &cat2, dcat2);
   Act d_ll = slice_act(dcat2, 0, 48), d_up = slice_act(dcat2, 48, 256);
-  b.push([=](cudaStream_t s) { return relu_mask_inplace(d_ll.ptr, ll.ptr, d_ll.pixels(), 48, d_ll.ld, ll.ld, s); });
   Act dlow_extra = b.act(H4, W4, 256);
   b.dgrad(d_ll, c + ".project.0", c + ".project.1", 256, 48, 1, 1, 1, nullptr, nullptr, dlow_extra);
   Act daspp = b.act(h, w, 256);
@@ -313,21 +314,20 @@
   b.dgrad(daspp, c + ".aspp.project.0", c + ".aspp.project.1", 1280, 256, 1, 1, 1, nullptr, &cat5, dcat5);
   Act dfeat = b.act(h, w, 2048);
   {
+    Act d4 = slice_act(dcat5, 1024, 256);
+    Act dg2 = b.act(1, 1, 256), dpooled = b.act(1, 1, 2048);
+    float* rb = static_cast<float*>(b.bump.take(static_cast<size_t>(B) * 2048 * sizeof(float)));
+    b.push([=](cudaStream_t s) { return sum_hw(d4.ptr, nullptr, dg2.ptr, B, h * w, 256, d4.ld, s); });
+    b.dgrad(dg2, c + ".aspp.convs.4.1", c + ".aspp.convs.4.2", 2048, 256, 1, 1, 1, nullptr, nullptr, dpooled);
+    b.push([=](cudaStream_t s) { return gap_bwd_rowbias(dpooled.ptr, rb, B, h * w, 2048, s); });
     Act d0 = slice_act(dcat5, 0, 256);
     b.dgrad(d0, c + ".aspp.convs.0.0", c + ".aspp.convs.0.1", 2048, 256, 1, 1, 1, nullptr, nullptr, dfeat);
     for (int k = 0; k < 3; ++k) {
       Act dk = slice_act(dcat5, 256 * (k + 1), 256);
+      const bool last = k == 2;
       b.dgrad(dk, c + ".aspp.convs." + std::to_string(k + 1) + ".0", c + ".aspp.convs." + std::to_string(k + 1) + ".1", 2048, 256,
-              3, 1, rates[k], &dfeat, nullptr, dfeat);
-    }
-    Act d4 = slice_act(dcat5, 1024, 256);
-    Act dg2 = b.act(1, 1, 256), dpooled = b.act(1, 1, 2048);
-    b.push([=](cudaStream_t s) { return sum_hw(d4.ptr, nullptr, dg2.ptr, B, h * w, 256, d4.ld, s); });
-    b.dgrad(dg2, c + ".aspp.convs.4.1", c + ".aspp.convs.4.2", 2048, 256, 1, 1, 1, nullptr, nullptr, dpooled);
-    b.push([=](cudaStream_t s) {
-      if (int e = gap_bwd_add(dpooled.ptr, dfeat.ptr, B, h * w, 2048, dfeat.ld, s)) return e;
-      return relu_mask_inplace(dfeat.ptr, feat.ptr, dfeat.pixels(), 2048, dfeat.ld, feat.ld, s);
-    });
+              3, 1, rates[k], &dfeat, last ? &feat : nullptr, dfeat, nullptr, false, last ? rb : nullptr, 2048);
+    }
   }
   Act g = dfeat;
   for (int i = static_cast<int>(blocks.size()) - 1; i >= 0; --i) {
@@ -368,16 +368,15 @@
     const Act gp = g;
     const float* sc = bn1.first;
     const int P = net->grad_pool;
-    float* weff = nullptr;
+    __nv_bfloat16* frag = nullptr;
     if (!dry && P > 1) {
-      const int R = P / 2 + 3;
-      weff = static_cast<float*>(b.arena->alloc(static_cast<size_t>(R) * R * 192 * sizeof(float)));
-      if (!weff) return 1;
-      if (int e = conv1_dgrad_weff(w_conv1, sc, weff, P, st)) return e;
+      frag = static_cast<__nv_bfloat16*>(b.arena->alloc(stem_bwd_frag_bytes(P)));
+      if (!frag) return 1;
+      if (int e = conv1_dgrad_weff(w_conv1, sc, frag, P, st)) return e;
     }
     b.push([=](cudaStream_t s) {
+      if (P > 1) return stem_bwd_pooled(gp.ptr, pool_idx, p1.ptr, frag, n->grad_out, B, H, W, P, s);
       if (int e = maxpool_bwd(gp.ptr, pool_idx, c1.ptr, dc1.ptr, B, H2, W2, 64, s)) return e;
-      if (P > 1) return conv1_dgrad_pooled(dc1.ptr, weff, n->grad_out, B, H, W, P, s);
       return conv1_dgrad(dc1.ptr, w_conv1, sc, n->grad_out, B, H, W, 64, s);
     });
     net->flops_bwd += 2.0 * B * H2 * W2 * 147.0 * 64;
diff --git a/weatherconverter_b200/csrc/seg_kernels.cu b/weatherconverter_b200/csrc/seg_kernels.cu
--- a/weatherconverter_b200/csrc/seg_kernels.cu
+++ b/weatherconverter_b200/csrc/seg_kernels.cu
@@ -155,17 +155,10 @@
     v[static_cast<size_t>(b) * C + c] = __float2bfloat16_rn(s);
   }
 }
-__global__ void gap_bwd_add_kernel(const __nv_bfloat16* __restrict__ g, __nv_bfloat16* __restrict__ dx, int B, int HW, int C, int ld) {
-  pdl_prologue();
-  const size_t total = static_cast<size_t>(B) * HW * C;
+__global__ void gap_bwd_rowbias_kernel(const __nv_bfloat16* __restrict__ g, float* __restrict__ rb, int n, int HW) {
+  pdl_prologue();
   const float inv = 1.f / HW;
-  for (size_t i = blockIdx.x * static_cast<size_t>(blockDim.x) + threadIdx.x; i < total;
-       i += static_cast<size_t>(gridDim.x) * blockDim.x) {
-    const int c = static_cast<int>(i % C);
-    const size_t p = i / C, b = p / HW;
-    __nv_bfloat16* d = dx + p * ld + c;
-    *d = __float2bfloat16_rn(__bfloat162float(*d) + __bfloat162float(g[b * C + c]) * inv);
-  }
+  for (int i = blockIdx.x * blockDim.x + threadIdx.x; i < n; i += gridDim.x * blockDim.x) rb[i] = __bfloat162float(g[i]) * inv;
 }
 
 __device__ __forceinline__ void bilinear_src(int dst, float scale, int in_size, int& i0, int& i1, float& l1) {
@@ -552,79 +545,133 @@
   }
 }
 
-__global__ void conv1_dgrad_weff_kernel(const float* __restrict__ w, const float* __restrict__ scale, float* __restrict__ weff,
+__global__ void conv1_dgrad_weff_kernel(const float* __restrict__ w, const float* __restrict__ scale, __nv_bfloat16* __restrict__ frag,
                                         int P) {
   pdl_prologue();
   const int R = P / 2 + 3;
-  const int total = R * R * 3 * 64;
+  const int total = R * R * 4 * 32 * 4;
   for (int idx = blockIdx.x * blockDim.x + threadIdx.x; idx < total; idx += gridDim.x * blockDim.x) {
-    const int o = idx & 63, c = (idx >> 6) % 3, rs = idx / 192, s_ = rs % R - 1, r_ = rs / R - 1;
-    float acc = 0.f;
-    for (int j = 0; j < P; ++j) {
-      const int ky = j + 3 - 2 * r_;
-      if (ky < 0 || ky > 6) continue;
-      for (int i = 0; i < P; ++i) {
-        const int kx = i + 3 - 2 * s_;
-        if (kx < 0 || kx > 6) continue;
-        acc += w[((static_cast<size_t>(o) * 3 + c) * 7 + ky) * 7 + kx];
-      }
-    }
-    weff[idx] = acc * (scale ? scale[o] : 1.f) / static_cast<float>(P * P);
-  }
-}
-
-__global__ void __launch_bounds__(128)
-conv1_dgrad_pooled_kernel(const __nv_bfloat16* __restrict__ dz, const float* __restrict__ weff, float* __restrict__ out, int B,
-                          int Ho, int Wo, int P) {
-  pdl_prologue();
-  extern __shared__ float sw[];
-  const int R = P / 2 + 3, half = P / 2;
-  for (int i = threadIdx.x; i < R * R * 192; i += blockDim.x) sw[i] = weff[i];
+    const int hf = idx & 1, reg = (idx >> 1) & 1, lane = (idx >> 2) & 31, kc = (idx >> 7) & 3, rs = idx >> 9;
+    const int n = lane >> 2, o = 16 * kc + 2 * (lane & 3) + hf + 8 * reg;
+    float v = 0.f;
+    if (n < 6) {
+      const int c = n >> 1, s_ = rs % R - 1, r_ = rs / R - 1;
+      float acc = 0.f;
+      for (int j = 0; j < P; ++j) {
+        const int ky = j + 3 - 2 * r_;
+        if (ky < 0 || ky > 6) continue;
+        for (int i = 0; i < P; ++i) {
+          const int kx = i + 3 - 2 * s_;
+          if (kx < 0 || kx > 6) continue;
+          acc += w[((static_cast<size_t>(o) * 3 + c) * 7 + ky) * 7 + kx];
+        }
+      }
+      const float weff = acc * (scale ? scale[o] : 1.f) / static_cast<float>(P * P);
+      const float hi = __bfloat162float(__float2bfloat16_rn(weff));
+      v = (n & 1) ? weff - hi : hi;
+    }
+    frag[idx] = __float2bfloat16_rn(v);
+  }
+}
+
+constexpr int kSbTX = 16;
+inline int stem_bwd_rows(int P) { return P <= 4 ? 8 : (P == 6 ? 4 : 2); }
+inline size_t stem_bwd_smem(int P) {
+  const int half = P / 2, R = half + 3;
+  return static_cast<size_t>(R) * R * 4 * 32 * 8 + static_cast<size_t>(half * stem_bwd_rows(P) + 3) * (half * kSbTX + 3) * 128;
+}
+
+__device__ __forceinline__ void ldmatrix_x4(uint32_t addr, uint32_t (&a)[4]) {
+  asm volatile("ldmatrix.sync.aligned.m8n8.x4.shared.b16 {%0,%1,%2,%3}, [%4];"
+               : "=r"(a[0]), "=r"(a[1]), "=r"(a[2]), "=r"(a[3]) : "r"(addr) : "memory");
+}
+__device__ __forceinline__ void mma_bf16_16816(float (&d)[4], const uint32_t (&a)[4], uint2 b) {
+  asm volatile("mma.sync.aligned.m16n8k16.row.col.f32.bf16.bf16.f32 {%0,%1,%2,%3}, {%4,%5,%6,%7}, {%8,%9}, {%0,%1,%2,%3};"
+               : "+f"(d[0]), "+f"(d[1]), "+f"(d[2]), "+f"(d[3])
+               : "r"(a[0]), "r"(a[1]), "r"(a[2]), "r"(a[3]), "r"(b.x), "r"(b.y));
+}
+
+__global__ void __launch_bounds__(256)
+stem_bwd_pooled_kernel(const __nv_bfloat16* __restrict__ gp, const uint8_t* __restrict__ idx, const __nv_bfloat16* __restrict__ p1,
+                       const uint2* __restrict__ wfrag, float* __restrict__ out, int H2, int W2, int P, int TY) {
+  pdl_prologue();
+  extern __shared__ __align__(128) uint8_t sb_smem[];
+  const int half = P / 2, R = half + 3, ntap = R * R;
+  const int FW = half * kSbTX + 3, FH = half * TY + 3;
+  const int Ho = H2 / 2, Wo = W2 / 2, Hp = 2 * H2 / P, Wp = 2 * W2 / P;
+  uint2* sfrag = reinterpret_cast<uint2*>(sb_smem);
+  uint8_t* sdz = sb_smem + static_cast<size_t>(ntap) * 4 * 32 * 8;
+  const int b = blockIdx.z, Y0 = blockIdx.y * TY, X0 = blockIdx.x * kSbTX;
+  for (int i = threadIdx.x; i < ntap * 128; i += blockDim.x) sfrag[i] = __ldg(wfrag + i);
+  const int iy0 = half * Y0 - 1, ix0 = half * X0 - 1;
+  for (int i = threadIdx.x; i < FH * FW * 8; i += blockDim.x) {
+    const int c8 = i & 7, pix = i >> 3, fy = pix / FW, fx = pix - fy * FW;
+    const int iy = iy0 + fy, ix = ix0 + fx;
+    float acc[8];
+    bool pos[8];
+#pragma unroll
+    for (int j = 0; j < 8; ++j) { acc[j] = 0.f; pos[j] = false; }
+    if (iy >= 0 && iy < H2 && ix >= 0 && ix < W2) {
+      for (int oy = iy / 2; oy <= (iy + 1) / 2; ++oy) {
+        if (oy >= Ho) continue;
+        const int ky = iy - (2 * oy - 1);
+        for (int ox = ix / 2; ox <= (ix + 1) / 2; ++ox) {
+          if (ox >= Wo) continue;
+          const int kx = ix - (2 * ox - 1);
+          const uint32_t tap = static_cast<uint32_t>(ky * 3 + kx);
+          const size_t q = ((static_cast<size_t>(b) * Ho + oy) * Wo + ox) * 64 + c8 * 8;
+          const uint2 ii = __ldg(reinterpret_cast<const uint2*>(idx + q));
+          const uint4 g = __ldg(reinterpret_cast<const uint4*>(gp + q));
+          const uint4 m = __ldg(reinterpret_cast<const uint4*>(p1 + q));
+          const uint32_t* gw = &g.x;
+          const uint32_t* mw = &m.x;
+#pragma unroll
+          for (int j = 0; j < 8; ++j) {
+            const uint32_t t = ((j < 4 ? ii.x : ii.y) >> (8 * (j & 3))) & 0xffu;
+            const float2 f = unpack_bf16(gw[j >> 1]), fm = unpack_bf16(mw[j >> 1]);
+            if (t == tap) {
+              acc[j] += (j & 1) ? f.y : f.x;
+              pos[j] = ((j & 1) ? fm.y : fm.x) > 0.f;
+            }
+          }
+        }
+      }
+    }
+    uint4 o;
+    o.x = pack_bf16(pos[0] ? acc[0] : 0.f, pos[1] ? acc[1] : 0.f);
+    o.y = pack_bf16(pos[2] ? acc[2] : 0.f, pos[3] ? acc[3] : 0.f);
+    o.z = pack_bf16(pos[4] ? acc[4] : 0.f, pos[5] ? acc[5] : 0.f);
+    o.w = pack_bf16(pos[6] ? acc[6] : 0.f, pos[7] ? acc[7] : 0.f);
+    *reinterpret_cast<uint4*>(sdz + static_cast<size_t>(pix) * 128 + ((c8 ^ ((fx / half) & 7)) << 4)) = o;
+  }
   __syncthreads();
-  const int Hp = Ho / half, Wp = Wo / half;
-  const size_t total = static_cast<size_t>(B) * Hp * Wp;
-  for (size_t i = blockIdx.x * static_cast<size_t>(blockDim.x) + threadIdx.x; i < total;
-       i += static_cast<size_t>(gridDim.x) * blockDim.x) {
-    const int X = static_cast<int>(i % Wp), Y = static_cast<int>((i / Wp) % Hp), b = static_cast<int>(i / (static_cast<size_t>(Wp) * Hp));
-    float2 a0 = make_float2(0.f, 0.f), a1 = a0, a2 = a0;
-    for (int r = 0; r < R; ++r) {
-      const int oy = half * Y + r - 1;
-      if (oy < 0 || oy >= Ho) continue;
-      for (int s_ = 0; s_ < R; ++s_) {
-        const int ox = half * X + s_ - 1;
-        if (ox < 0 || ox >= Wo) continue;
-        const uint4* zp = reinterpret_cast<const uint4*>(dz + ((static_cast<size_t>(b) * Ho + oy) * Wo + ox) * 64);
-        const float4* wp = reinterpret_cast<const float4*>(sw + (r * R + s_) * 192);
-#pragma unroll
-        for (int o8 = 0; o8 < 8; ++o8) {
-          const uint4 u = __ldg(zp + o8);
-          const float2 f0 = unpack_bf16(u.x), f1 = unpack_bf16(u.y), f2 = unpack_bf16(u.z), f3 = unpack_bf16(u.w);
-          const float4 w0a = wp[o8 * 2], w0b = wp[o8 * 2 + 1];
-          const float4 w1a = wp[16 + o8 * 2], w1b = wp[16 + o8 * 2 + 1];
-          const float4 w2a = wp[32 + o8 * 2], w2b = wp[32 + o8 * 2 + 1];
-          a0 = ffma2(f0, make_float2(w0a.x, w0a.y), a0); a0 = ffma2(f1, make_float2(w0a.z, w0a.w), a0);
-          a0 = ffma2(f2, make_float2(w0b.x, w0b.y), a0); a0 = ffma2(f3, make_float2(w0b.z, w0b.w), a0);
-          a1 = ffma2(f0, make_float2(w1a.x, w1a.y), a1); a1 = ffma2(f1, make_float2(w1a.z, w1a.w), a1);
-          a1 = ffma2(f2, make_float2(w1b.x, w1b.y), a1); a1 = ffma2(f3, make_float2(w1b.z, w1b.w), a1);
-          a2 = ffma2(f0, make_float2(w2a.x, w2a.y), a2); a2 = ffma2(f1, make_float2(w2a.z, w2a.w), a2);
-          a2 = ffma2(f2, make_float2(w2b.x, w2b.y), a2); a2 = ffma2(f3, make_float2(w2b.z, w2b.w), a2);
-        }
-      }
-    }
-    const size_t plane = static_cast<size_t>(Hp) * Wp, o = static_cast<size_t>(b) * 3 * plane + static_cast<size_t>(Y) * Wp + X;
-    out[o] = a0.x + a0.y; out[o + plane] = a1.x + a1.y; out[o + 2 * plane] = a2.x + a2.y;
-  }
-}
-
-__global__ void relu_mask_kernel(__nv_bfloat16* __restrict__ d, const __nv_bfloat16* __restrict__ m, size_t npix, int C,
-                                 int ldd, int ldm) {
-  pdl_prologue();
-  const size_t total = npix * C;
-  for (size_t i = blockIdx.x * static_cast<size_t>(blockDim.x) + threadIdx.x; i < total;
-       i += static_cast<size_t>(gridDim.x) * blockDim.x) {
-    const size_t p = i / C;
-    const int c = static_cast<int>(i % C);
-    if (!(__bfloat162float(m[p * ldm + c]) > 0.f)) d[p * ldd + c] = __float2bfloat16_rn(0.f);
+  const int warp = threadIdx.x >> 5, lane = threadIdx.x & 31;
+  const int Y = Y0 + warp;
+  if (Y >= Hp) return;
+  const int arow = (lane & 7) + ((lane >> 3) & 1) * 8;
+  const int ahi = lane >> 4;
+  const uint32_t dz_base = smem_u32(sdz);
+  float acc[2][4] = {{0.f, 0.f, 0.f, 0.f}, {0.f, 0.f, 0.f, 0.f}};
+  for (int r = 0; r < R; ++r) {
+    const int fy = half * warp + r;
+    for (int s = 0; s < R; ++s) {
+      const int fx = half * arow + s;
+      const uint32_t prow = dz_base + static_cast<uint32_t>(fy * FW + fx) * 128u;
+      const int key = (arow + s / half) & 7;
+      const uint2* bf = sfrag + (r * R + s) * 128 + lane;
+#pragma unroll
+      for (int kc = 0; kc < 4; ++kc) {
+        uint32_t a[4];
+        ldmatrix_x4(prow + (static_cast<uint32_t>((2 * kc + ahi) ^ key) << 4), a);
+        mma_bf16_16816(acc[kc & 1], a, bf[kc * 32]);
+      }
+    }
+  }
+  const int gx = lane >> 2, c = lane & 3;
+  if (c < 3) {
+    float* o = out + ((static_cast<size_t>(b) * 3 + c) * Hp + Y) * Wp + X0;
+    if (X0 + gx < Wp) o[gx] = (acc[0][0] + acc[1][0]) + (acc[0][1] + acc[1][1]);
+    if (X0 + gx + 8 < Wp) o[gx + 8] = (acc[0][2] + acc[1][2]) + (acc[0][3] + acc[1][3]);
   }
 }
 
@@ -689,9 +736,9 @@
   WC_LAUNCH_CHECK();
   return 0;
 }
-int gap_bwd_add(const __nv_bfloat16* g, __nv_bfloat16* dx, int B, int HW, int C, int ld, cudaStream_t st) {
-  ProfScope prof(kProfOther, st, 0);
-  launch_k(gap_bwd_add_kernel, grid_for(static_cast<size_t>(B) * HW * C), 256, 0, st, g, dx, B, HW, C, ld);
+int gap_bwd_rowbias(const __nv_bfloat16* g, float* rb, int B, int HW, int C, cudaStream_t st) {
+  ProfScope prof(kProfOther, st, static_cast<double>(B) * C * 6.0);
+  launch_k(gap_bwd_rowbias_kernel, grid_for(static_cast<size_t>(B) * C), 256, 0, st, g, rb, B * C, HW);
   WC_LAUNCH_CHECK();
   return 0;
 }
@@ -769,28 +816,27 @@
   WC_LAUNCH_CHECK();
   return 0;
 }
-int conv1_dgrad_weff(const float* w, const float* scale, float* weff, int P, cudaStream_t st) {
-  launch_k(conv1_dgrad_weff_kernel, 8, 256, 0, st, w, scale, weff, P);
-  WC_LAUNCH_CHECK();
-  return 0;
-}
-int conv1_dgrad_pooled(const __nv_bfloat16* dz, const float* weff, float* out, int B, int H, int W, int P, cudaStream_t st) {
-  WC_REQUIRE(P >= 2 && P % 2 == 0 && P <= 8 && H % P == 0 && W % P == 0, "pooled stem gradient needs an even pool <= 8 dividing H and W");
-  const int R = P / 2 + 3;
-  const size_t smem = static_cast<size_t>(R) * R * 192 * sizeof(float);
+size_t stem_bwd_frag_bytes(int P) { return static_cast<size_t>(P / 2 + 3) * (P / 2 + 3) * 4 * 32 * 8; }
+int conv1_dgrad_weff(const float* w, const float* scale, __nv_bfloat16* frag, int P, cudaStream_t st) {
+  WC_REQUIRE(P >= 2 && P % 2 == 0 && P <= 8, "pooled stem gradient needs an even pool <= 8");
+  launch_k(conv1_dgrad_weff_kernel, 8, 256, 0, st, w, scale, frag, P);
+  WC_LAUNCH_CHECK();
+  return 0;
+}
+int stem_bwd_pooled(const __nv_bfloat16* gp, const uint8_t* idx, const __nv_bfloat16* p1, const __nv_bfloat16* frag, float* out, int B,
+                    int H, int W, int P, cudaStream_t st) {
+  WC_REQUIRE(P >= 2 && P % 2 == 0 && P <= 8 && H % P == 0 && W % P == 0 && H % 4 == 0 && W % 4 == 0,
+             "pooled stem gradient needs an even pool <= 8 dividing H and W");
+  const size_t smem = stem_bwd_smem(P);
   static size_t attr = 0;
   if (smem > 48 * 1024 && smem > attr) {
-    WC_CHECK_CUDA(cudaFuncSetAttribute(conv1_dgrad_pooled_kernel, cudaFuncAttributeMaxDynamicSharedMemorySize, static_cast<int>(smem)));
+    WC_CHECK_CUDA(cudaFuncSetAttribute(stem_bwd_pooled_kernel, cudaFuncAttributeMaxDynamicSharedMemorySize, static_cast<int>(smem)));
     attr = smem;
   }
-  ProfScope prof(kProfBoundaryConv, st, static_cast<double>(B) * (12.0 * (H / P) * (W / P) + 2.0 * (H / 2) * (W / 2) * 64));
-  launch_k(conv1_dgrad_pooled_kernel, grid_for(static_cast<size_t>(B) * (H / P) * (W / P), 128), 128, smem, st, dz, weff, out, B, H / 2, W / 2, P);
-  WC_LAUNCH_CHECK();
-  return 0;
-}
-int relu_mask_inplace(__nv_bfloat16* d, const __nv_bfloat16* m, size_t npix, int C, int ldd, int ldm, cudaStream_t st) {
-  ProfScope prof(kProfOther, st, 0);
-  launch_k(relu_mask_kernel, grid_for(npix * C), 256, 0, st, d, m, npix, C, ldd, ldm);
+  const int TY = stem_bwd_rows(P), Hp = H / P, Wp = W / P;
+  ProfScope prof(kProfBoundaryConv, st, static_cast<double>(B) * (12.0 * Hp * Wp + 5.0 * (H / 4) * (W / 4) * 64));
+  launch_k(stem_bwd_pooled_kernel, dim3((Wp + kSbTX - 1) / kSbTX, (Hp + TY - 1) / TY, B), 32 * TY, smem, st, gp, idx, p1,
+           reinterpret_cast<const uint2*>(frag), out, H / 2, W / 2, P, TY);
   WC_LAUNCH_CHECK();
   return 0;
 }
diff --git a/weatherconverter_b200/csrc/wc_api.cu b/weatherconverter_b200/csrc/wc_api.cu
--- a/weatherconverter_b200/csrc/wc_api.cu
+++ b/weatherconverter_b200/csrc/wc_api.cu
@@ -52,6 +52,10 @@
                         cudaStream_t st);
 int conv1_dgrad(const __nv_bfloat16* dz, const float* w, const float* scale, float* dx, int B, int H, int W, int Cout,
                 cudaStream_t st);
+size_t stem_bwd_frag_bytes(int P);
+int conv1_dgrad_weff(const float* w, const float* scale, __nv_bfloat16* frag, int P, cudaStream_t st);
+int stem_bwd_pooled(const __nv_bfloat16* gp, const uint8_t* idx, const __nv_bfloat16* p1, const __nv_bfloat16* frag, float* out, int B,
+                    int H, int W, int P, cudaStream_t st);
 int groupnorm_silu_bwd(const __nv_bfloat16* x, const __nv_bfloat16* dy, __nv_bfloat16* dx, int B, int HW, int C, int ld,
                        int ldd, int ldo, const float* gamma, const float* beta, float eps, int silu, const void* stats,
                        const __nv_bfloat16* add1, int lda1, const __nv_bfloat16* add2, int lda2, float* dgamma, float* dbeta,
@@ -245,6 +249,20 @@
 int wc_conv1_dgrad(const wc_bf16* dz, const float* weight, const float* scale, float* dx, int batch, int H, int W, void* stream) {
   return conv1_dgrad(BF(dz), weight, scale, dx, batch, H, W, 64, S(stream));
 }
+int wc_stem_bwd_pooled(const wc_bf16* gp, const uint8_t* idx, const wc_bf16* p1, const float* weight, const float* scale, float* out,
+                       int batch, int H, int W, int P, void* stream) {
+  WC_REQUIRE(P >= 2 && P % 2 == 0 && P <= 8, "pool must be 2, 4, 6 or 8");
+  cudaStream_t st = S(stream);
+  void* frag = nullptr;
+  WC_CHECK_CUDA(cudaMalloc(&frag, stem_bwd_frag_bytes(P)));
+  int e = conv1_dgrad_weff(weight, scale, static_cast<__nv_bfloat16*>(frag), P, st);
+  if (!e) e = stem_bwd_pooled(BF(gp), idx, BF(p1), static_cast<const __nv_bfloat16*>(frag), out, batch, H, W, P, st);
+  const cudaError_t se = cudaStreamSynchronize(st);
+  cudaFree(frag);
+  if (e) return e;
+  WC_CHECK_CUDA(se);
+  return 0;
+}
 int wc_conv_in(const float* x, const float* weight, const float* bias, const float* scale, const float* shift,
                wc_bf16* y, int batch, int H, int W, int Cout, int K, int stride, int pad, int ldy, int relu,
                void* stream) {
```

New measurement: 3.014, median of 6. 1.1% higher.
